# clovaai/assembled-cnn

Hardware: AMD Instinct MI355X
Metric: images/sec Assemble-ResNet-50 224^2 bf16 train (higher is better)
Workload: dtype bf16; 1 GPU; Assemble-ResNet-50 (BigLittle + SK + anti_alias sconv k=3 + resnet_d) bf16 train; per_gpu_batch=256, global_batch=256, image=224x224x3, num_classes=1001, parallelism=dp1

## Files before the change

### assembled_cnn_amd/csrc/conv_gemm1.hip

```cpp
#include "common.h"
#include "igemm_common.h"

using namespace asm_igemm;

namespace {

typedef __attribute__((address_space(3))) void* lptr_t;

template <int N>
__device__ __forceinline__ void wait_vm() {
  asm volatile("s_waitcnt vmcnt(%0)" ::"n"(N) : "memory");
}
template <int P, int RMAX>
__device__ __forceinline__ void wait_vm_steps(const int r) {
  if constexpr (RMAX <= 0) {
    wait_vm<0>();
  } else {
    if (r >= RMAX) wait_vm<P * RMAX>();
    else wait_vm_steps<P, RMAX - 1>(r);
  }
}

template <int BM, int BN, int BK, int WGM, int WGN, int NS>
struct Cfg1 {
  using C = Cfg<BM, BN, BK, WGM, WGN, false, true>;
  static constexpr int STAGE = (BM + BN) * C::ROWB;
  static constexpr int LDS = cmax(cmax(NS * STAGE, C::EPI), C::RED);
  static constexpr int P = C::XP + C::WP;
  static_assert(BN % C::RPP == 0, "every wave issues the same number of pieces (the vmcnt immediates count them)");
  static_assert(C::RPP % 16 == 0, "the source-side swizzle must not depend on the pass");
  static_assert(NS >= 2 && P * (NS - 2) <= 63, "vmcnt is a 6-bit counter");
  static_assert(LDS <= 160 * 1024, "lds");
};

template <int BM, int BN, int BK, int WGM, int WGN, bool STATS, int NS, bool PFA, bool POOL, bool BNRED = false>
__global__ __launch_bounds__(64 * WGM * WGN) void igemm1_kernel(IGemmArgs p) {
  using C = Cfg<BM, BN, BK, WGM, WGN, false, STATS>;
  using C1 = Cfg1<BM, BN, BK, WGM, WGN, NS>;
  constexpr int CPR = C::CPR, RPP = C::RPP, XP = C::XP, WP = C::WP, ROWB = C::ROWB, STAGE = C1::STAGE, P = C1::P;
  constexpr int TM = C::TM, TN = C::TN, WTM = C::WTM, WTN = C::WTN;
  constexpr int KK = BK / 16;
  static_assert(KK >= 2 && KK % 2 == 0, "fragment double buffer: the last group of a step lives in buffer 1");

  extern __shared__ __attribute__((aligned(16))) unsigned char smem[];

  const int tid = threadIdx.x;
  const int lane = tid & 63;
  const int wave = tid >> 6;
  const int wm = wave / WGN, wn = wave % WGN;

  int logical;
  {
    const int nb = p.n_blocks, q = nb >> 3, r = nb & 7;
    const int bid = blockIdx.x, xcd = bid & 7, idx = bid >> 3;
    logical = (xcd < r ? xcd * (q + 1) : r * (q + 1) + (xcd - r) * q) + idx;
  }
  const int tile_m = (int)fd_div((unsigned)logical, p.fd_ntn);
  const int tile_n = logical - tile_m * p.n_tiles_n;

  const __amdgpu_buffer_rsrc_t rx = make_rsrc(p.x, p.x_bytes);
  const __amdgpu_buffer_rsrc_t rw = make_rsrc(p.w, p.w_bytes);

  const int chunk = tid % CPR;
  const int r0 = tid / CPR;
  const int csw = (chunk ^ swz<BK>(r0)) << 3;
  const bool c_ok = csw < p.Ci;

  unsigned vx[XP];
#pragma unroll
  for (int j = 0; j < XP; ++j) {
    const int m = tile_m * BM + r0 + j * RPP;
    bool ok = c_ok && m < p.M;
    const unsigned img = fd_div((unsigned)m, p.fd_howo);
    const unsigned rem = (unsigned)m - img * (unsigned)p.HoWo;
    const unsigned ho = fd_div(rem, p.fd_wo);
    const unsigned wo = rem - ho * (unsigned)p.Wo;
    int nh = (int)ho * p.so - p.pad, nw = (int)wo * p.so - p.pad_w;
    if (p.sd == 2) {
      ok = ok && (((nh | nw) & 1) == 0);
      nh >>= 1;
      nw >>= 1;
    }
    ok = ok && ((unsigned)nh < (unsigned)p.Hi) && ((unsigned)nw < (unsigned)p.Wi);
    vx[j] = ok ? (img * (unsigned)p.x_img_pitch + (unsigned)nh * (unsigned)p.x_row_pitch +
                  (unsigned)nw * (unsigned)p.x_pix_pitch + (unsigned)csw) * 2u
               : ASM_OOB;
  }
  unsigned vw[WP];
#pragma unroll
  for (int j = 0; j < WP; ++j) {
    const int n = tile_n * BN + r0 + j * RPP;
    vw[j] = (c_ok && n < p.Co) ? ((unsigned)n * (unsigned)p.w_row_pitch + (unsigned)csw) * 2u : ASM_OOB;
  }

  const int wrow0 = wave * (64 / CPR);
  const unsigned wtap = (unsigned)p.wt0 * (unsigned)p.Ci * 2u;
  auto issue = [&](int stage, unsigned kb) {
    unsigned char* xs = smem + stage * STAGE;
    unsigned char* ws = xs + BM * ROWB;
#pragma unroll
    for (int j = 0; j < XP; ++j)
      __builtin_amdgcn_raw_ptr_buffer_load_lds(rx, (lptr_t)(xs + (j * RPP + wrow0) * ROWB), 16, (int)vx[j], (int)kb, 0, 0);
#pragma unroll
    for (int j = 0; j < WP; ++j)
      __builtin_amdgcn_raw_ptr_buffer_load_lds(rw, (lptr_t)(ws + (j * RPP + wrow0) * ROWB), 16, (int)vw[j],
                                               (int)(kb + wtap), 0, 0);
  };

  f32x16 acc[TN][TM];
#pragma unroll
  for (int a = 0; a < TN; ++a)
#pragma unroll
    for (int b = 0; b < TM; ++b)
#pragma unroll
      for (int i = 0; i < 16; ++i) acc[a][b][i] = 0.f;

  const int l31 = lane & 31, lhi = lane >> 5;
  unsigned fwo[KK], fxo[KK];
#pragma unroll
  for (int kk = 0; kk < KK; ++kk) {
    const int ch = kk * 2 + lhi;
    const int rw_ = wn * WTN + l31, rx_ = wm * WTM + l31;
    fwo[kk] = BM * ROWB + rw_ * ROWB + ((ch ^ swz<BK>(rw_)) << 4);
    fxo[kk] = rx_ * ROWB + ((ch ^ swz<BK>(rx_)) << 4);
  }
  bf16x8 fwb[2][TN], fxb[2][TM];
  auto load_frags = [&](int stage, const int kk, const int buf) {
    const unsigned char* sb = smem + stage * STAGE;
#pragma unroll
    for (int a = 0; a < TN; ++a) fwb[buf][a] = *reinterpret_cast<const bf16x8*>(sb + fwo[kk] + a * 32 * ROWB);
#pragma unroll
    for (int b = 0; b < TM; ++b) fxb[buf][b] = *reinterpret_cast<const bf16x8*>(sb + fxo[kk] + b * 32 * ROWB);
  };
  auto mma = [&](const int buf) {
#pragma unroll
    for (int a = 0; a < TN; ++a)
#pragma unroll
      for (int b = 0; b < TM; ++b)
        acc[a][b] = __builtin_amdgcn_mfma_f32_32x32x16_bf16(fwb[buf][a], fxb[buf][b], acc[a][b], 0, 0, 0);
  };

  const int nk = p.kchunks;
#pragma unroll
  for (int s = 0; s < NS - 1; ++s)
    if (s < nk) issue(s, (unsigned)(s * BK * 2));
#pragma unroll
  for (int a = 0; a < TN; ++a) fwb[1][a] = bf16x8{0, 0, 0, 0, 0, 0, 0, 0};
#pragma unroll
  for (int b = 0; b < TM; ++b) fxb[1][b] = bf16x8{0, 0, 0, 0, 0, 0, 0, 0};
  int cur = 0;
  unsigned kb_next = (unsigned)((NS - 1) * BK * 2);
#pragma unroll 1
  for (int kc = 0; kc < nk; ++kc) {
    wait_vm_steps<P, NS - 2>(nk - 1 - kc);
    asm volatile("s_waitcnt lgkmcnt(0)\n\ts_barrier" ::: "memory");
    load_frags(cur, 0, 0);
    mma(1);
    if (kc + NS - 1 < nk) {
      int nst = cur + NS - 1;
      if (nst >= NS) nst -= NS;
      issue(nst, kb_next);
    }
#pragma unroll
    for (int kk = 0; kk + 1 < KK; ++kk) {
      load_frags(cur, kk + 1, (kk + 1) & 1);
      mma(kk & 1);
    }
    cur = cur + 1 == NS ? 0 : cur + 1;
    kb_next += BK * 2;
  }
  mma(1);
  __syncthreads();

  igemm_epilogue<C, BM, BN, WTM, WTN, TM, TN, false, STATS, PFA, POOL, false, BNRED>(p, acc, smem, tile_m, tile_n, tid, wm, wn, l31, lhi);
}

template <int BM, int BN, int BK, int WGM, int WGN, bool STATS, int NS, bool PFA, bool POOL, bool BNRED = false>
int launch1_one(const IGemmArgs& a, hipStream_t st) {
  using C1 = Cfg1<BM, BN, BK, WGM, WGN, NS>;
  auto kern = igemm1_kernel<BM, BN, BK, WGM, WGN, STATS, NS, PFA, POOL, BNRED>;
  static bool attr_done[ASM_MAX_DEVICES] = {};
  if (hipError_t e = asm_ensure_dyn_lds(kern, C1::LDS, attr_done); e != hipSuccess)
    ASM_FAIL(ASM_EHIP, "igemm1_kernel: dynamic LDS opt-in: %s", hipGetErrorString(e));
  ASM_LAUNCH(kern, dim3(a.n_blocks), dim3(64 * WGM * WGN), C1::LDS, st, a);
  ASM_CHECK_LAUNCH("igemm1_kernel");
  return ASM_OK;
}

template <int BM, int BN, int BK, int WGM, int WGN, int NS>
int launch1(const ConvLaunch& L, const IGemmArgs& a, hipStream_t st) {
  switch (L.epi) {
    case EPI_BNRED: return launch1_one<BM, BN, BK, WGM, WGN, true, NS, false, false, true>(a, st);
    case EPI_STATS: return launch1_one<BM, BN, BK, WGM, WGN, true, NS, false, false>(a, st);
    case EPI_POOL: return launch1_one<BM, BN, BK, WGM, WGN, false, NS, false, true>(a, st);
    case EPI_PFA: return launch1_one<BM, BN, BK, WGM, WGN, false, NS, true, false>(a, st);
    case EPI_PLAIN: return launch1_one<BM, BN, BK, WGM, WGN, false, NS, false, false>(a, st);
  }
  return conv_no_variant("igemm1_kernel", L.epi);
}

struct Config {
  int code;
  ConvTile t;
  int (*launch)(const ConvLaunch&, const IGemmArgs&, hipStream_t);
};
constexpr Config kConfigs[] = {
    {1, {128, 128, 64, 2, 2}, launch1<128, 128, 64, 2, 2, 2>},
    {5, {128, 128, 32, 2, 2}, launch1<128, 128, 32, 2, 2, 3>},
    {8, {256, 128, 64, 4, 2}, launch1<256, 128, 64, 4, 2, 3>},
    {10, {128, 128, 32, 2, 2}, launch1<128, 128, 32, 2, 2, 2>},
    {11, {128, 64, 64, 2, 2}, launch1<128, 64, 64, 2, 2, 2>},
    {12, {128, 64, 32, 2, 2}, launch1<128, 64, 32, 2, 2, 3>},
    {13, {128, 64, 32, 2, 2}, launch1<128, 64, 32, 2, 2, 2>},
    {14, {256, 128, 32, 4, 2}, launch1<256, 128, 32, 4, 2, 3>},
    {16, {128, 256, 32, 2, 2}, launch1<128, 256, 32, 2, 2, 2>},
};

struct AutoRow {
  int kind, M, Ci, Co, code;
};
constexpr AutoRow kAuto[] = {
    {0, 802816,   32,   64, 13}, {0, 802816,   32,  128, 13}, {0, 802816,   64,   32, 12}, {0, 802816,   64,  128, 10},
    {0, 802816,  128,  256, 10}, {0, 802816,  256,   64, 12}, {0, 200704,   64,  256, 10}, {0, 200704,  256,   64, 12},
    {0, 200704,  256,  128,  5}, {0, 200704,  256,  256,  5}, {0, 200704,  256,  512, 10}, {0, 200704,  512,  128,  5},
    {0,  50176,  128,  512, 10}, {0,  50176,  256,  512, 10}, {0,  50176,  256, 1024, 10}, {0,  50176,  512,  128, 14},
    {0,  50176,  512,  256, 16}, {0,  50176,  512,  512, 10}, {0,  50176,  512, 1024, 10}, {0,  50176, 1024,  256, 16},
    {0,  50176, 1024,  512, 16}, {0,  50176, 1024, 1024, 14}, {0,  12544,  256, 1024, 16}, {0,  12544,  512, 1024, 14},
    {0,  12544,  512, 2048, 10}, {0,  12544, 1024,  256,  5}, {0,  12544, 2048,  512,  8}, {1, 802816,   32,   64, 12},
    {1, 802816,   64,   32, 12}, {1, 802816,   64,   64, 11}, {1, 802816,   64,  256, 16}, {1, 802816,  128,   32, 13},
    {1, 802816,  128,   64, 13}, {1, 802816,  256,  128,  5}, {1, 200704,   64,  256,  5}, {1, 200704,  128,  256,  5},
    {1, 200704,  128,  512,  5}, {1, 200704,  256,   64, 12}, {1, 200704,  256,  256, 10}, {1, 200704,  512,  256,  5},
    {1,  50176,  128,  512, 10}, {1,  50176,  256,  512, 10}, {1,  50176,  256, 1024, 14}, {1,  50176,  512,  128,  1},
    {1,  50176,  512,  512, 10}, {1,  50176,  512, 1024, 10}, {1,  50176, 1024,  256, 16}, {1,  50176, 1024,  512, 14},
    {1,  50176, 1024, 1024, 10}, {1,  12544,  256, 1024, 14}, {1,  12544,  512, 2048, 10}, {1,  12544, 1024,  256,  8},
    {1,  12544, 1024,  512,  8}, {1,  12544, 2048,  512,  8}, {1,  12544, 2048, 1024, 16}, {2, 802816,   64,  256, 14},
    {2, 200704,   64,  256, 13}, {2, 200704,  128,  256, 12}, {2, 200704,  128,  512, 14}, {2,  50176,  128,  512, 12},
    {2,  50176,  256,  512, 12}, {2,  50176,  256, 1024, 13}, {2,  50176,  512, 1024, 14}, {2,  12544,  256, 1024, 14},
    {2,  12544,  512, 2048, 14},
    {0, 802816,   64,  256, 10}, {1, 802816,  256,   64, 11}, {0, 802816,  256,  128, 14}, {1, 802816,  128,  256, 14},
    {2, 802816,  128,  256, 14}, {0, 200704,  128,  512, 10}, {1, 200704,  512,  128,  5}, {0, 200704,  512,  256,  5},
    {1, 200704,  256,  512, 10}, {2, 200704,  256,  512, 14}, {0, 401408,   64,   64, 12}, {1, 100352,  256,   64, 12},
    {0, 100352,  256,   64, 12}, {1, 100352,   64,  256,  5}, {2, 100352,   64,  256, 13}, {0, 401408,   64,  256, 10},
    {0, 401408,  256,  256,  5}, {1, 401408,  256,  256, 14}, {0, 100352,  256,  256, 10}, {1, 100352,  256,  256, 10},
    {0, 401408,  256,   64, 12}, {1, 401408,   64,  256,  5}, {2, 401408,   64,  256, 14}, {0,  25088,  256,  512, 16},
    {1,  25088,  512,  256,  8}, {0, 100352,  256,  128, 14}, {1, 100352,  128,  256, 12}, {2, 100352,  128,  256, 12},
    {0,  25088,  128,  512, 10}, {1,  25088,  512,  128, 11}, {0,  25088,  512,  128,  5}, {1,  25088,  128,  512, 14},
    {2,  25088,  128,  512, 12}, {0, 100352,  256,  512, 10}, {0, 100352,  128,  512, 10}, {1, 100352,  512,  128, 14},
    {1, 100352,  128,  512, 10}, {2, 100352,  128,  512, 12}, {0, 100352,  512,  512, 14}, {1, 100352,  512,  512, 14},
    {1,   6272, 1024,  512,  5}, {0,  25088,  512,  256,  8}, {1,  25088,  256,  512, 14}, {2,  25088,  256,  512, 14},
    {1,   6272, 1024,  256, 12}, {0,   6272, 1024,  256, 11}, {1,   6272,  256, 1024,  8}, {0,  25088,  256, 1024, 10},
    {1,  25088, 1024,  256,  8}, {0,  25088, 1024,  256,  8}, {1,  25088,  256, 1024, 10}, {2,  25088,  256, 1024, 10},
    {1,   6272, 2048, 1024,  8}, {1,   6272, 2048,  512,  5}, {0,   6272, 2048,  512,  5},
};

int auto_cfg(const IGemmArgs& a, bool stats) {
  if (a.so != 1 || a.sd != 1 || a.y_strided || a.pool_dy) return 0;
  const int kind = a.tsign < 0 ? (a.addend ? 2 : 1) : (stats ? 0 : -1);
  for (const AutoRow& r : kAuto)
    if (r.kind == kind && r.M == a.M && r.Ci == a.Ci && r.Co == a.Co) return r.code;
  return 0;
}

}

int asm_gemm1_config(const IGemmArgs& a, bool out_f32, bool stats, ConvTile* t) {
  if (out_f32 || a.R != 1 || a.S != 1 || a.bn_scale) return 0;
  const int g = asm_tune().gemm1;
  const int code = g < 0 ? auto_cfg(a, stats) : g;
  for (const Config& c : kConfigs)
    if (c.code == code && (a.Ci % c.t.bk == 0 || a.Ci <= c.t.bk)) { *t = c.t; return code; }
  return 0;
}

int asm_gemm1_launch(const ConvLaunch& L, const IGemmArgs& a, hipStream_t st) {
  for (const Config& c : kConfigs)
// ... 4 lines not shown
```

### assembled_cnn_amd/csrc/conv_igemm.hip

```cpp
#include "common.h"
#include "igemm_common.h"

using namespace asm_igemm;

int asm_gemm1_config(const IGemmArgs& a, bool out_f32, bool stats, ConvTile* t);
int asm_gemm1_launch(const ConvLaunch& L, const IGemmArgs& a, hipStream_t st);
bool asm_igemm8_covers(const IGemmArgs& a, bool out_f32);
int asm_igemm8_launch(const ConvLaunch& L, const IGemmArgs& a, hipStream_t st);

namespace {

__device__ __attribute__((aligned(16))) unsigned g_zero16[4] = {0u, 0u, 0u, 0u};


template <int BM, int BN, int BK, int WGM, int WGN, bool OUT_F32, bool STATS, bool BNRED = false>
__global__ __launch_bounds__(64 * WGM * WGN) void igemm_kernel(IGemmArgs p) {
  using C = Cfg<BM, BN, BK, WGM, WGN, OUT_F32, STATS>;
  constexpr int NT = C::NT, CPR = C::CPR, RPP = C::RPP, XP = C::XP, WP = C::WP, ROWB = C::ROWB, STAGE = C::STAGE;
  constexpr int TM = C::TM, TN = C::TN, WTM = C::WTM, WTN = C::WTN;

  extern __shared__ __attribute__((aligned(16))) unsigned char smem[];

  const int tid = threadIdx.x;
  const int lane = tid & 63;
// ... 72 lines not shown
    const int tap0 = (kt_r * p.S + kt_s) * p.Ci + kt_c * BK;
#pragma unroll
    for (int j = 0; j < WP; ++j) {
      const int row = r0 + j * RPP;
      if (j * RPP + wrow0 < BN) {
        const int c = ((chunk ^ swz<BK>(row)) << 3);
        const bool ok = live && (kt_c * BK + c < p.Ci) && (wb[j] >= 0);
        const unsigned off = (unsigned)(wb[j] + tap0 + c) * 2u;
        const unsigned char* src = ok ? reinterpret_cast<const unsigned char*>(p.w) + off
                                      : reinterpret_cast<const unsigned char*>(g_zero16);
        __builtin_amdgcn_global_load_lds((gptr_t)src, (lptr_t)(ws + (j * RPP + wrow0) * ROWB), 16, 0, 0);
      }
    }
    if (++kt_s == p.S) {
      kt_s = 0;
      if (++kt_r == p.R) {
        kt_r = 0;
        ++kt_c;
      }
    }
  };

  f32x16 acc[TN][TM];
#pragma unroll
  for (int a = 0; a < TN; ++a)
#pragma unroll
    for (int b = 0; b < TM; ++b)
#pragma unroll
      for (int i = 0; i < 16; ++i) acc[a][b][i] = 0.f;

  const int KT = p.R * p.S * p.kchunks;
  const int l31 = lane & 31, lhi = lane >> 5;

  auto compute = [&](int stage) {
    const unsigned char* xs = smem + stage * STAGE;
    const unsigned char* ws = xs + BM * ROWB;
#pragma unroll
    for (int kk = 0; kk < BK / 16; ++kk) {
      const int ch = kk * 2 + lhi;
      bf16x8 fw[TN], fx[TM];
#pragma unroll
      for (int a = 0; a < TN; ++a) {
        const int row = wn * WTN + a * 32 + l31;
        fw[a] = *reinterpret_cast<const bf16x8*>(ws + row * ROWB + ((ch ^ swz<BK>(row)) << 4));
      }
#pragma unroll
      for (int b = 0; b < TM; ++b) {
        const int row = wm * WTM + b * 32 + l31;
        fx[b] = *reinterpret_cast<const bf16x8*>(xs + row * ROWB + ((ch ^ swz<BK>(row)) << 4));
      }
#pragma unroll
      for (int a = 0; a < TN; ++a)
#pragma unroll
        for (int b = 0; b < TM; ++b)
          acc[a][b] = __builtin_amdgcn_mfma_f32_32x32x16_bf16(fw[a], fx[b], acc[a][b], 0, 0, 0);
    }
  };

  issue_tile(0, true);
  asm volatile("s_waitcnt vmcnt(0)" ::: "memory");
  __syncthreads();
#pragma unroll 1
  for (int kt = 0; kt < KT; ++kt) {
    const int cur = kt & 1;
    if (kt + 1 < KT) issue_tile(cur ^ 1, true);
    compute(cur);
    asm volatile("s_waitcnt vmcnt(0)" ::: "memory");
    __syncthreads();
  }

  igemm_epilogue<C, BM, BN, WTM, WTN, TM, TN, OUT_F32, STATS, false, false, false, BNRED>(p, acc, smem, tile_m, tile_n, tid, wm, wn, l31, lhi);
}

template <int BM, int BN, int BK, int WGM, int WGN, bool OUT_F32, bool STATS, int NS>
struct Cfg2 {
  using C = Cfg<BM, BN, BK, WGM, WGN, OUT_F32, STATS>;
  static constexpr int WROWS = BN;
  static constexpr int STAGE = (BM + WROWS) * C::ROWB;
  static constexpr int LDS = cmax(cmax(NS * STAGE, C::EPI), C::RED);
  static_assert(LDS <= 160 * 1024, "lds");
};

template <int BM, int BN, int BK, int WGM, int WGN, bool OUT_F32, bool STATS, int R, int S, int NS, bool PFA = false, bool POOL = false,
          int SCHED = 0, bool BNRED = false>
__global__ __launch_bounds__(64 * WGM * WGN) void igemm2_kernel(IGemmArgs p) {
  using C = Cfg<BM, BN, BK, WGM, WGN, OUT_F32, STATS>;
  using C2 = Cfg2<BM, BN, BK, WGM, WGN, OUT_F32, STATS, NS>;
  constexpr int CPR = C::CPR, RPP = C::RPP, XP = C::XP, WP = C::WP, ROWB = C::ROWB, STAGE = C2::STAGE;
  constexpr int TM = C::TM, TN = C::TN, WTM = C::WTM, WTN = C::WTN;
  constexpr int NTAP = R * S;
  static_assert(RPP % 16 == 0, "the source-side swizzle must not depend on the pass");
  typedef __attribute__((address_space(3))) void* lptr_t;

  extern __shared__ __attribute__((aligned(16))) unsigned char smem[];

  const int tid = threadIdx.x;
  const int lane = tid & 63;
  const int wave = tid >> 6;
  const int wm = wave / WGN, wn = wave % WGN;

  int logical;
  {
    const int nb = p.n_blocks, q = nb >> 3, r = nb & 7;
    const int bid = blockIdx.x, xcd = bid & 7, idx = bid >> 3;
    logical = (xcd < r ? xcd * (q + 1) : r * (q + 1) + (xcd - r) * q) + idx;
  }
  const int tile_m0 = (int)fd_div((unsigned)logical, p.fd_ntn);
  const int tile_n = logical - tile_m0 * p.n_tiles_n;
  const int tile_m = tile_m0 + p.m_tile0;

  const __amdgpu_buffer_rsrc_t rx = make_rsrc(p.x, p.x_bytes);
  const __amdgpu_buffer_rsrc_t rw = make_rsrc(p.w, p.w_bytes);

  const int chunk = tid % CPR;
  const int r0 = tid / CPR;
  const int csw = (chunk ^ swz<BK>(r0)) << 3;
  const bool c_ok = csw < p.Ci;

  unsigned vx[XP][NTAP];
#pragma unroll
  for (int j = 0; j < XP; ++j) {
    const int m = tile_m * BM + r0 + j * RPP;
    const bool live = c_ok && m < p.M;
    const unsigned img = fd_div((unsigned)m, p.fd_howo);
    const unsigned rem = (unsigned)m - img * (unsigned)p.HoWo;
    const unsigned ho = fd_div(rem, p.fd_wo);
    const unsigned wo = rem - ho * (unsigned)p.Wo;
    const int bh = (int)ho * p.so - p.pad, bw = (int)wo * p.so - p.pad_w;
    const unsigned base = img * (unsigned)p.x_img_pitch + (unsigned)csw;
    unsigned roff[R], coff[S];
    bool rok[R], cok[S];
#pragma unroll
    for (int r = 0; r < R; ++r) {
      int nh = bh + p.tsign * r;
      bool ok = live;
      if (p.sd == 2) {
        ok = ok && ((nh & 1) == 0);
        nh >>= 1;
      }
      rok[r] = ok && ((unsigned)nh < (unsigned)p.Hi);
      roff[r] = base + (unsigned)nh * (unsigned)p.x_row_pitch;
    }
#pragma unroll
    for (int q = 0; q < S; ++q) {
      int nw = bw + p.tsign * q;
      bool ok = true;
      if (p.sd == 2) {
        ok = ((nw & 1) == 0);
        nw >>= 1;
      }
      cok[q] = ok && ((unsigned)nw < (unsigned)p.Wi);
      coff[q] = (unsigned)nw * (unsigned)p.x_pix_pitch;
    }
#pragma unroll
    for (int r = 0; r < R; ++r)
#pragma unroll
      for (int q = 0; q < S; ++q) vx[j][r * S + q] = (rok[r] && cok[q]) ? (roff[r] + coff[q]) * 2u : ASM_OOB;
  }
  unsigned vw[WP];
#pragma unroll
  for (int j = 0; j < WP; ++j) {
    const int row = r0 + j * RPP;
    const int n = tile_n * BN + row;
    vw[j] = (c_ok && row < BN && n < p.Co) ? ((unsigned)n * (unsigned)p.w_row_pitch + (unsigned)csw) * 2u : ASM_OOB;
  }

  const int wrow0 = wave * (64 / CPR);
// ... 407 lines not shown
  };

  unsigned fxo[TM], fwo[TN];
#pragma unroll
  for (int b = 0; b < TM; ++b) {
    const int row = wm * WTM + b * 32 + l31;
    fxo[b] = (unsigned)(((row >> 4) * HW_ + (row & 15)) * RB + lhi * 16);
  }
#pragma unroll
  for (int a = 0; a < TN; ++a) fwo[a] = (unsigned)((wn * WTN + a * 32 + l31) * WROWB);
  const int wsw = swz<CI>(wn * WTN + l31);

  u32x4 hv[HP];
  if (t_begin < t_end) load_halo(t_begin, hv);
  asm volatile("s_waitcnt vmcnt(0)" ::: "memory");

#pragma unroll 1
  for (int tile = t_begin; tile < t_end; ++tile) {
    __syncthreads();
    store_halo(hv);
    __syncthreads();
    if (tile + 1 < t_end) load_halo(tile + 1, hv);

    f32x16 acc[TN][TM];
#pragma unroll
    for (int a = 0; a < TN; ++a)
#pragma unroll
      for (int b = 0; b < TM; ++b)
#pragma unroll
        for (int i = 0; i < 16; ++i) acc[a][b][i] = 0.f;
#pragma unroll
    for (int t = 0; t < 9; ++t) {
      const int r = t / 3, q = t - r * 3;
      const int hoff = (p.tsign > 0 ? (r * HW_ + q) : ((2 - r) * HW_ + (2 - q))) * RB;
#pragma unroll
      for (int kk = 0; kk < KK; ++kk) {
        bf16x8 fw[TN], fx[TM];
#pragma unroll
        for (int a = 0; a < TN; ++a)
          fw[a] = *reinterpret_cast<const bf16x8*>(ws + t * WTAP + fwo[a] + (((kk * 2 + lhi) ^ wsw) << 4));
#pragma unroll
        for (int b = 0; b < TM; ++b) fx[b] = *reinterpret_cast<const bf16x8*>(xs + fxo[b] + hoff + kk * 32);
#pragma unroll
        for (int a = 0; a < TN; ++a)
#pragma unroll
          for (int b = 0; b < TM; ++b) acc[a][b] = __builtin_amdgcn_mfma_f32_32x32x16_bf16(fw[a], fx[b], acc[a][b], 0, 0, 0);
      }
    }
    __syncthreads();
    const int img = tile / tpi, trem = tile - img * tpi;
    const int ty = trem / tiles_x, tx = trem - ty * tiles_x;
    const int patch_base = (img * p.Hi + ty * 8) * p.Wi + tx * 16;
    igemm_epilogue<C, 128, KO, WTM, WTN, TM, TN, false, STATS>(p, acc, xs, tile, 0, tid, wm, wn, l31, lhi, patch_base);
  }
}

template <int KO, int CI, int WGM, int WGN, bool STATS>
int launch_halo_one(const IGemmArgs& a, hipStream_t st) {
  using H = HaloCfg<KO, CI>;
  auto kern = conv_halo_kernel<KO, CI, WGM, WGN, STATS>;
  static bool attr_done[ASM_MAX_DEVICES] = {};
  if (hipError_t e = asm_ensure_dyn_lds(kern, H::LDS, attr_done); e != hipSuccess)
    ASM_FAIL(ASM_EHIP, "conv_halo_kernel: dynamic LDS opt-in: %s", hipGetErrorString(e));
  ASM_LAUNCH(kern, dim3(a.n_blocks), dim3(256), H::LDS, st, a);
  ASM_CHECK_LAUNCH("conv_halo_kernel");
  return ASM_OK;
}

template <int KO, int CI, int WGM, int WGN>
int launch_halo(const ConvLaunch& L, const IGemmArgs& a, hipStream_t st) {
  return L.epi == EPI_STATS ? launch_halo_one<KO, CI, WGM, WGN, true>(a, st) : launch_halo_one<KO, CI, WGM, WGN, false>(a, st);
}

bool halo_covers(const IGemmArgs& a, bool out_f32) {
  if (out_f32 || a.R != 3 || a.S != 3 || a.so != 1 || a.sd != 1 || a.y_strided || a.bn_scale) return false;
  if (a.Hi % 8 || a.Wi % 16 || a.M != (a.HoWo / a.Wo) * a.Wo * (a.M / a.HoWo) || a.HoWo != a.Hi * a.Wi) return false;
  if (a.x_pix_pitch != a.Ci || a.x_row_pitch != a.Wi * a.Ci || a.x_img_pitch != a.Hi * a.Wi * a.Ci) return false;
  if (!((a.tsign > 0 && a.pad == 1 && a.pad_w == 1) || (a.tsign < 0 && a.pad == -1 && a.pad_w == -1))) return false;
  if (a.wt0 != 0 || a.wtr != 3 || a.wts != 1) return false;
  return (a.Ci == 32 || a.Ci == 64) && (a.Co == 32 || a.Co == 64);
}

template <int BM, int BN, int BK, int WGM, int WGN, bool OUT_F32, bool STATS, int R, int S, int NS = 2, bool PFA = false, bool POOL = false,
          int SCHED = 0, bool BNRED = false>
int launch2_one(const IGemmArgs& a, hipStream_t st) {
  using C = Cfg2<BM, BN, BK, WGM, WGN, OUT_F32, STATS, NS>;
  constexpr int NTHR = 64 * WGM * WGN;
  if constexpr (SCHED == 0 && BK == 64 && BN >= 128 && !OUT_F32 && !POOL && ((R == 3 && S == 3) || (R == 1 && S == 1))) {
    if (R == 3) return launch2_one<BM, BN, BK, WGM, WGN, OUT_F32, STATS, R, S, NS, PFA, POOL, 1>(a, st);
  }
  auto kern = igemm2_kernel<BM, BN, BK, WGM, WGN, OUT_F32, STATS, R, S, NS, PFA, POOL, SCHED, BNRED>;
  static bool attr_done[ASM_MAX_DEVICES] = {};
  if (hipError_t e = asm_ensure_dyn_lds(kern, C::LDS, attr_done); e != hipSuccess)
    ASM_FAIL(ASM_EHIP, "igemm2_kernel: dynamic LDS opt-in: %s", hipGetErrorString(e));
  ASM_LAUNCH(kern, dim3(a.n_blocks), dim3(NTHR), C::LDS, st, a);
  ASM_CHECK_LAUNCH("igemm2_kernel");
  return ASM_OK;
}

constexpr unsigned igemm2_variants(int R, int S, int BM, int BN, int BK) {
  if (R == 1 && S == 1)
    return epi_bit(EPI_F32) | epi_bit(EPI_BNRED) | epi_bit(EPI_STATS) | epi_bit(EPI_POOL) | epi_bit(EPI_PFA) | epi_bit(EPI_PLAIN);
  if (R == 3 && S == 3) return epi_bit(EPI_STATS) | epi_bit(EPI_PFA) | epi_bit(EPI_PLAIN);
  if ((R == 1 && S == 2) || (R == 2 && S == 1) || (R == 2 && S == 2)) return epi_bit(EPI_PLAIN);
  if ((R == 7 || R == 3) && S == 1 && BK == 32 && BM == 128 && BN <= 64) return epi_bit(EPI_STATS) | epi_bit(EPI_PLAIN);
  return 0;
}

template <int BM, int BN, int BK, int WGM, int WGN, int R, int S>
int launch2_rs(const ConvLaunch& L, const IGemmArgs& a, hipStream_t st) {
  constexpr unsigned has = igemm2_variants(R, S, BM, BN, BK);
  if constexpr ((has >> EPI_F32) & 1)
    if (L.epi == EPI_F32) return launch2_one<BM, BN, BK, WGM, WGN, true, false, R, S>(a, st);
  if constexpr ((has >> EPI_BNRED) & 1)
    if (L.epi == EPI_BNRED) return launch2_one<BM, BN, BK, WGM, WGN, false, true, R, S, 2, false, false, 0, true>(a, st);
  if constexpr ((has >> EPI_STATS) & 1)
    if (L.epi == EPI_STATS) return launch2_one<BM, BN, BK, WGM, WGN, false, true, R, S>(a, st);
  if constexpr ((has >> EPI_POOL) & 1)
    if (L.epi == EPI_POOL) return launch2_one<BM, BN, BK, WGM, WGN, false, false, R, S, 2, false, true>(a, st);
  if constexpr ((has >> EPI_PFA) & 1)
    if (L.epi == EPI_PFA) return launch2_one<BM, BN, BK, WGM, WGN, false, false, R, S, 2, true>(a, st);
  if constexpr ((has >> EPI_PLAIN) & 1)
    if (L.epi == EPI_PLAIN) return launch2_one<BM, BN, BK, WGM, WGN, false, false, R, S>(a, st);
  return conv_no_variant("igemm2_kernel", L.epi);
}

template <int BM, int BN, int BK, int WGM, int WGN>
struct Launch2 {
  static int run(const ConvLaunch& L, const IGemmArgs& a, hipStream_t st) {
    if (a.R == 1 && a.S == 1) return launch2_rs<BM, BN, BK, WGM, WGN, 1, 1>(L, a, st);
    if (a.R == 3 && a.S == 3) return launch2_rs<BM, BN, BK, WGM, WGN, 3, 3>(L, a, st);
    if (a.R == 1 && a.S == 2) return launch2_rs<BM, BN, BK, WGM, WGN, 1, 2>(L, a, st);
    if (a.R == 2 && a.S == 1) return launch2_rs<BM, BN, BK, WGM, WGN, 2, 1>(L, a, st);
    if (a.R == 2 && a.S == 2) return launch2_rs<BM, BN, BK, WGM, WGN, 2, 2>(L, a, st);
    if (a.R == 7 && a.S == 1) return launch2_rs<BM, BN, BK, WGM, WGN, 7, 1>(L, a, st);
    if (a.R == 3 && a.S == 1) return launch2_rs<BM, BN, BK, WGM, WGN, 3, 1>(L, a, st);
    return conv_no_variant("igemm2_kernel", L.epi);
  }
};

template <int BM, int BN, int BK, int WGM, int WGN, bool OUT_F32, bool STATS, bool BNRED = false>
int launch_one(const IGemmArgs& a, hipStream_t st) {
  using C = Cfg<BM, BN, BK, WGM, WGN, OUT_F32, STATS>;
  auto kern = igemm_kernel<BM, BN, BK, WGM, WGN, OUT_F32, STATS, BNRED>;
  static bool attr_done[ASM_MAX_DEVICES] = {};
  if (hipError_t e = asm_ensure_dyn_lds(kern, C::LDS, attr_done); e != hipSuccess)
    ASM_FAIL(ASM_EHIP, "igemm_kernel: dynamic LDS opt-in: %s", hipGetErrorString(e));
  ASM_LAUNCH(kern, dim3(a.n_blocks), dim3(C::NT), C::LDS, st, a);
  ASM_CHECK_LAUNCH("igemm_kernel");
  return ASM_OK;
}

template <int BM, int BN, int BK, int WGM, int WGN>
struct LaunchGeneral {
  static int run(const ConvLaunch& L, const IGemmArgs& a, hipStream_t st) {
    switch (L.epi) {
      case EPI_F32: return launch_one<BM, BN, BK, WGM, WGN, true, false>(a, st);
      case EPI_BNRED: return launch_one<BM, BN, BK, WGM, WGN, false, true, true>(a, st);
      case EPI_STATS: return launch_one<BM, BN, BK, WGM, WGN, false, true>(a, st);
      case EPI_PLAIN: return launch_one<BM, BN, BK, WGM, WGN, false, false>(a, st);
    }
    return conv_no_variant("igemm_kernel", L.epi);
  }
};

template <template <int, int, int, int, int> class F>
int on_tile(const ConvLaunch& L, const IGemmArgs& a, hipStream_t st) {
  const ConvTile& t = L.t;
  if (t.bm == 256) return F<256, 256, 64, 4, 2>::run(L, a, st);
  if (t.bn == 32) return t.bk == 64 ? F<128, 32, 64, 4, 1>::run(L, a, st) : F<128, 32, 32, 4, 1>::run(L, a, st);
  if (t.bn == 64) return t.bk == 64 ? F<128, 64, 64, 2, 2>::run(L, a, st) : F<128, 64, 32, 2, 2>::run(L, a, st);
  return t.bk == 64 ? F<128, 128, 64, 2, 2>::run(L, a, st) : F<128, 128, 32, 2, 2>::run(L, a, st);
}

enum class ConvOut { bf16, f32, stats, bnred };

bool tile256(const IGemmArgs& a) {
  const int ftile = asm_tune().igemm_tile;
  if (ftile == 1) return false;
  if (ftile == 3 && a.Ci % 64 == 0) return true;
  const long long b256 = (long long)cdiv(a.M, 256) * cdiv(a.Co, 256);
  return a.Ci % 64 == 0 && (long long)a.R * a.S * a.Ci >= 512 && a.Co >= 256 && b256 >= 192;
}

ConvTile pick_tile(const IGemmArgs& a) {
  const long long t128 = (long long)cdiv(a.M, 128) * cdiv(a.Co, 128);
  const bool bk64 = a.Ci % 64 == 0 && (a.R * a.S > 1 || (a.Ci >= 256 && t128 <= 4000));
  if (a.Co <= 32) return bk64 ? ConvTile{128, 32, 64, 4, 1} : ConvTile{128, 32, 32, 4, 1};
  if (a.Co <= 64) return bk64 ? ConvTile{128, 64, 64, 2, 2} : ConvTile{128, 64, 32, 2, 2};
  if (tile256(a)) return ConvTile{256, 256, 64, 4, 2};
  return bk64 ? ConvTile{128, 128, 64, 2, 2} : ConvTile{128, 128, 32, 2, 2};
}

unsigned family_variants(int family, const IGemmArgs& a, const ConvTile& t) {
  switch (family) {
    case FAM_GENERAL: return epi_bit(EPI_F32) | epi_bit(EPI_BNRED) | epi_bit(EPI_STATS) | epi_bit(EPI_PLAIN);
    case FAM_IGEMM2: return igemm2_variants(a.R, a.S, t.bm, t.bn, t.bk);
    case FAM_HALO: return epi_bit(EPI_STATS) | epi_bit(EPI_PLAIN);
    case FAM_DENSE: return epi_bit(EPI_F32) | epi_bit(EPI_PLAIN);
    case FAM_GEMM1: return epi_bit(EPI_BNRED) | epi_bit(EPI_STATS) | epi_bit(EPI_POOL) | epi_bit(EPI_PFA) | epi_bit(EPI_PLAIN);
    default: return epi_bit(EPI_BNRED) | epi_bit(EPI_STATS) | epi_bit(EPI_PFA) | epi_bit(EPI_PLAIN);
  }
}

ConvLaunch tiled(int family, ConvTile t, const IGemmArgs& a, ConvOut out, int M, int m_tile0) {
  ConvLaunch L = {};
  L.family = family; L.t = t; L.M = M; L.m_tile0 = m_tile0;
  L.n_tiles_n = cdiv(a.Co, t.bn);
  L.n_blocks = (cdiv(M, t.bm) - m_tile0) * L.n_tiles_n;
  L.kchunks = cdiv(a.Ci, t.bk);
  const unsigned has = family_variants(family, a, t);
  const int pfa_env = asm_tune().igemm_pfa;
  const bool pfa = (has & epi_bit(EPI_PFA)) && a.addend != nullptr && !a.y_strided &&
                   (pfa_env >= 0 ? pfa_env != 0 : (t.bm == 256 || L.n_blocks <= 1024));
  const int want = out == ConvOut::f32 ? EPI_F32 : out == ConvOut::bnred ? EPI_BNRED : out == ConvOut::stats ? EPI_STATS
                   : a.pool_dy ? EPI_POOL : pfa ? EPI_PFA : EPI_PLAIN;
  L.epi = (has & epi_bit(want)) ? want : -1;
  if (family == FAM_IGEMM3) {
    L.nhb = a.Ci == 64 ? 1 : 2;
    L.hr = a.Ci == 64 && a.Wi > 30 ? 256 : 192;
  }
  return L;
}

ConvPlan single(const ConvLaunch& L) { return ConvPlan{1, {L, {}}, nullptr}; }
ConvPlan no_plan(const char* why) { return ConvPlan{0, {}, why}; }

bool dense_shaped(const IGemmArgs& a) {
  return a.Hi == 1 && a.Wi == 1 && a.HoWo == 1 && a.R == 1 && a.S == 1 && a.x_img_pitch == a.Ci && a.x_row_pitch == a.Ci &&
         a.x_pix_pitch == a.Ci;
}
bool dense_covers(const IGemmArgs& a, ConvOut out) {
  if (!asm_tune().dense_small || !dense_shaped(a) || a.Ci % 16 || (out != ConvOut::bf16 && out != ConvOut::f32)) return false;
  if (a.addend_mask || a.pool_dy || a.bn_scale || a.y_strided) return false;
  if (a.ldy % 4 || a.ldy > cdiv(a.Co, 32) * 32) return false;
  return asm_aligned16(a.x) && asm_aligned16(a.w) && asm_aligned16(a.y) && asm_aligned16(a.addend);
}

ConvPlan plan_conv(const IGemmArgs& a, ConvOut out) {
  const asm_tuning& tu = asm_tune();
  const bool f32 = out == ConvOut::f32, stats = out == ConvOut::stats || out == ConvOut::bnred;
  const bool k1 = a.R == 1 && a.S == 1;
  const bool bnred3 = out == ConvOut::bnred && !k1;
  if (dense_covers(a, out)) return single(tiled(FAM_DENSE, ConvTile{32, 32, 16, 1, 1}, a, out, a.M, 0));
  if (dense_shaped(a) && (a.pool_dy || out == ConvOut::bnred))
    return no_plan("conv dgrad: the fused input-gradient forms do not take a [N,1,1,C] layer");
  if (a.pool_dy && (tu.igemm_mode != 0 || out != ConvOut::bf16 || !k1 || a.y_strided))
    return no_plan("conv dgrad_pooled: only the 1x1 stride-1 igemm2 path folds an average-pool backward in");
  if (tu.igemm_mode == 0 && tu.igemm_tile == 0) {
    if (halo_covers(a, f32)) {
      if (bnred3) return no_plan("conv dgrad_bnred: no kernel with the batch-norm sums for this 3x3 layer");
      const int ko = a.Co, ci = a.Ci;
      ConvLaunch L = tiled(FAM_HALO, ConvTile{128, ko, ci, ko == 32 ? 4 : 2, ko == 32 ? 1 : 2}, a, out, a.M, 0);
      const int per_cu = ko == 32 ? (ci == 32 ? HaloCfg<32, 32>::PER_CU : HaloCfg<32, 64>::PER_CU)
                                  : (ci == 32 ? HaloCfg<64, 32>::PER_CU : HaloCfg<64, 64>::PER_CU);
      L.n_blocks = a.M / 128 < per_cu * 256 ? a.M / 128 : per_cu * 256;
      return single(L);
    }
    ConvTile t1;
    if (const int code = asm_gemm1_config(a, f32, stats, &t1)) {
      ConvLaunch L = tiled(FAM_GEMM1, t1, a, out, a.M, 0);
      L.gemm1 = code;
      return single(L);
    }
    const int h3 = tu.igemm3, h8 = tu.igemm8;
    const ConvTile t128 = {128, 128, 64, 2, 2};
    const bool big = tile256(a);
    const long long b256 = (long long)cdiv(a.M, 256) * cdiv(a.Co, 256);
    const bool to_igemm3 = h3 && b256 >= 768 && a.Ci <= 128;
    const bool cov3 = h3 && igemm3_covers(a, f32);
    if (((h8 == 1 && big && !to_igemm3) || h8 == 2) && asm_igemm8_covers(a, f32)) {
      const ConvTile t8 = {256, 256, 64, 2, 4};
      const int cus = asm_num_cus();
      const int nt8 = cdiv(a.Co, 256), mt8 = cdiv(a.M, 256);
      const long long n8 = (long long)nt8 * mt8;
      const int m_full = (int)((n8 / cus) * cus / nt8);
      const long long rem = n8 - (long long)m_full * nt8;
      const double small = 4 * rem <= cus ? 0.3 : 0.5 * (double)((4 * rem + 2 * cus - 1) / (2 * cus));
      const double split_cost = (double)((long long)m_full * nt8 / cus) + small, whole_cost = (double)((n8 + cus - 1) / cus);
      if (h8 == 1 && m_full > 0 && rem > 0 && split_cost < whole_cost - 0.15 && (cov3 || !bnred3)) {
        return ConvPlan{2, {tiled(FAM_IGEMM8, t8, a, out, m_full * 256, 0),
                            tiled(cov3 ? FAM_IGEMM3 : FAM_IGEMM2, t128, a, out, a.M, m_full * 2)},
                        nullptr};
      }
      return single(tiled(FAM_IGEMM8, t8, a, out, a.M, 0));
    }
    if (cov3 && (h3 == 2 || !big || to_igemm3)) return single(tiled(FAM_IGEMM3, t128, a, out, a.M, 0));
  }
  if (bnred3) return no_plan("conv dgrad_bnred: no kernel with the batch-norm sums for this 3x3 layer");
  const ConvTile t = pick_tile(a);
  if (tu.igemm_mode == 0) {
    const ConvLaunch L = tiled(FAM_IGEMM2, t, a, out, a.M, 0);
    if (L.epi >= 0 && (a.Ci % t.bk == 0 || a.Ci <= t.bk)) return single(L);
    if (a.pool_dy) return no_plan("conv dgrad_pooled: no igemm2 instantiation for this shape");
  }
  return single(tiled(FAM_GENERAL, t, a, out, a.M, 0));
}

int run_plan(const ConvPlan& p, IGemmArgs a, hipStream_t st) {
  if (p.n == 0) ASM_FAIL(ASM_ENOTSUP, "%s", p.why);
  a.fd_howo = make_fastdiv((unsigned)a.HoWo);
  a.fd_wo = make_fastdiv((unsigned)a.Wo);
  for (int i = 0; i < p.n; ++i) {
    const ConvLaunch& L = p.l[i];
    a.M = L.M; a.m_tile0 = L.m_tile0; a.n_tiles_n = L.n_tiles_n; a.n_blocks = L.n_blocks; a.kchunks = L.kchunks;
    a.fd_ntn = make_fastdiv((unsigned)L.n_tiles_n);
    int rc;
    switch (L.family) {
      case FAM_GENERAL: rc = on_tile<LaunchGeneral>(L, a, st); break;
      case FAM_GEMM1: rc = asm_gemm1_launch(L, a, st); break;
      case FAM_IGEMM2: rc = on_tile<Launch2>(L, a, st); break;
      case FAM_IGEMM3: rc = L.nhb == 2 ? launch3<192, 2>(L, a, st) : L.hr == 192 ? launch3<192, 1>(L, a, st) : launch3<256, 1>(L, a, st); break;
      case FAM_HALO:
        rc = L.t.bn == 32 ? (L.t.bk == 64 ? launch_halo<32, 64, 4, 1>(L, a, st) : launch_halo<32, 32, 4, 1>(L, a, st))
                          : (L.t.bk == 64 ? launch_halo<64, 64, 2, 2>(L, a, st) : launch_halo<64, 32, 2, 2>(L, a, st));
        break;
      case FAM_IGEMM8: rc = asm_igemm8_launch(L, a, st); break;
      case FAM_DENSE:
        rc = asm_dense_small_launch(a.x, a.Ci, a.w, a.Ci, a.M, a.Co, a.Ci, a.y, a.ldy, L.epi == EPI_F32, a.addend, st);
        break;
      default: ASM_FAIL(ASM_EINVAL, "conv: no kernel family %d", L.family);
    }
    if (rc != ASM_OK) return rc;
  }
  asm_last_conv_kernel = p.l[p.n - 1].family;
  return ASM_OK;
}

int check_desc(const asm_conv_desc* d) {
  ASM_REQUIRE(d != nullptr, "conv: null descriptor");
  ASM_REQUIRE(d->N > 0 && d->H > 0 && d->W > 0 && d->C > 0 && d->K > 0 && d->R > 0 && d->S > 0,
              "conv: non-positive dimension");
  ASM_REQUIRE(d->C % 8 == 0, "conv: C=%d must be a multiple of 8", d->C);
  ASM_REQUIRE(d->stride == 1 || d->stride == 2, "conv: stride %d not supported", d->stride);
  ASM_REQUIRE(d->Ho > 0 && d->Wo > 0, "conv: bad output size");
  ASM_REQUIRE(d->pad >= 0 && d->pad < 64, "conv: bad pad");
  return ASM_OK;
}

}

static inline int64_t img_pitch(const asm_conv_desc* d) {
  return d->x_img_pitch ? d->x_img_pitch : (int64_t)d->H * d->W * d->C;
}
static inline int row_pitch(const asm_conv_desc* d) { return d->x_row_pitch ? d->x_row_pitch : d->W * d->C; }
static inline int pix_pitch(const asm_conv_desc* d) { return d->x_pix_pitch ? d->x_pix_pitch : d->C; }

extern "C" int asm_debug_last_conv_kernel(void) { return asm_last_conv_kernel; }

extern "C" int asm_conv2d_stats_blocks(const asm_conv_desc* d) {
  if (!d) return ASM_EINVAL;
  return cdiv(d->N * d->Ho * d->Wo, STATS_BM);
}

static int fprop_impl(const asm_conv_desc* d, const void* x, const void* w, void* y, float* stats_partial,
                      const float* bn_scale, const float* bn_shift, const void* residual, int relu, void* stream) {
  if (int e = check_desc(d)) return e;
  ASM_REQUIRE(x && w && y, "conv fprop: null pointer");
  const int64_t xelems = (int64_t)d->N * img_pitch(d);
  ASM_REQUIRE(xelems * 2 < (int64_t)ASM_OOB, "conv fprop: input larger than 2 GiB");
  const int ldy = d->ldy ? d->ldy : d->K;
  ASM_REQUIRE(ldy % (d->out_f32 ? 4 : 8) == 0 && ldy >= d->K, "conv fprop: bad ldy %d", ldy);
  ASM_REQUIRE(!(stats_partial && d->out_f32), "conv fprop: fused statistics need bf16 output");
  IGemmArgs a = {};
  a.x = x; a.w = w; a.y = y; a.addend = residual; a.stats = stats_partial;
  a.x_bytes = (unsigned)(xelems * 2);
  a.w_bytes = (unsigned)((int64_t)d->K * d->R * d->S * d->C * 2);
  a.M = d->N * d->Ho * d->Wo;
  a.Hi = d->H; a.Wi = d->W; a.Ci = d->C;
  a.Wo = d->Wo; a.HoWo = d->Ho * d->Wo;
  a.Co = d->K; a.ldy = ldy;
  a.R = d->R; a.S = d->S;
  a.so = d->stride; a.sd = 1; a.tsign = 1; a.pad = d->pad;
  a.pad_w = a.pad; a.wt0 = 0; a.wtr = a.S; a.wts = 1;
  a.bn_scale = bn_scale; a.bn_shift = bn_shift; a.bn_relu = relu;
  a.x_img_pitch = (int)img_pitch(d); a.x_row_pitch = row_pitch(d); a.x_pix_pitch = pix_pitch(d);
  a.w_row_pitch = d->R * d->S * d->C;
  const ConvOut out = d->out_f32 ? ConvOut::f32 : stats_partial ? ConvOut::stats : ConvOut::bf16;
  return run_plan(plan_conv(a, out), a, (hipStream_t)stream);
}

extern "C" int asm_conv2d_fprop(const asm_conv_desc* d, const void* x, const void* w, void* y,
                                float* stats_partial, void* stream) {
  return fprop_impl(d, x, w, y, stats_partial, nullptr, nullptr, nullptr, 0, stream);
}

extern "C" int asm_conv2d_fprop_bn(const asm_conv_desc* d, const void* x, const void* w, void* y, const float* scale,
                                   const float* shift, const void* residual, int relu, void* stream) {
  ASM_REQUIRE(d && scale && shift, "conv fprop_bn: null pointer");
  ASM_REQUIRE(!d->out_f32 && d->K % 8 == 0, "conv fprop_bn: needs bf16 output and K %% 8 == 0 (K=%d)", d->K);
  ASM_REQUIRE(d->ldy == 0 || d->ldy == d->K, "conv fprop_bn: padded output rows not supported");
  return fprop_impl(d, x, w, y, nullptr, scale, shift, residual, relu ? 1 : 0, stream);
}

struct PoolAdd {
  const void* dy;
  int k, stride, pad, Hp, Wp, cv;
};
struct BnRed {
  const void* y;
  const uint8_t* mask;
  float* partial;
};
static int dgrad_impl(const asm_conv_desc* d, const void* dy, const void* wt, const void* addend,
                      const uint8_t* addend_mask, void* dx, void* stream, const PoolAdd* pool = nullptr,
                      const BnRed* red = nullptr);
static IGemmArgs dgrad_args(const asm_conv_desc* d) {
  IGemmArgs a = {};
  a.x_bytes = (unsigned)((int64_t)d->N * d->Ho * d->Wo * d->K * 2);
  a.w_bytes = (unsigned)((int64_t)d->K * d->R * d->S * d->C * 2);
  a.M = d->N * d->H * d->W;
  a.Hi = d->Ho; a.Wi = d->Wo; a.Ci = d->K;
  a.Wo = d->W; a.HoWo = d->H * d->W;
  a.Co = d->C; a.ldy = d->C;
  a.R = d->R; a.S = d->S;
  a.so = 1; a.sd = d->stride; a.tsign = -1; a.pad = -d->pad; a.pad_w = a.pad;
  a.x_img_pitch = d->Ho * d->Wo * d->K; a.x_row_pitch = d->Wo * d->K; a.x_pix_pitch = d->K;
  a.w_row_pitch = d->R * d->S * d->K;
  a.wt0 = 0; a.wtr = a.S; a.wts = 1;
  return a;
}
static int dgrad_check(const asm_conv_desc* d) {
  if (int e = check_desc(d)) return e;
  ASM_REQUIRE(d->K % 8 == 0, "conv dgrad: K=%d must be a multiple of 8 (pad dy)", d->K);
  ASM_REQUIRE(d->x_img_pitch == 0 && d->x_row_pitch == 0 && d->x_pix_pitch == 0 && !d->out_f32,
              "conv dgrad: custom pitches / f32 output not supported");
  const int64_t dyelems = (int64_t)d->N * d->Ho * d->Wo * d->K;
  ASM_REQUIRE(dyelems * 2 < (int64_t)ASM_OOB, "conv dgrad: dy larger than 2 GiB");
  return ASM_OK;
}
bool asm_dgrad_s2_covers(const asm_conv_desc* d);
int asm_dgrad_s2_launch(const asm_conv_desc* d, const void* dy, const void* wt, const void* addend, const uint8_t* addend_mask,
                        void* dx, void* stream);

enum class DgradForm { conv, parity, s2 };
struct DgradPlan {
  DgradForm form;
  int nc;
  IGemmArgs cls[4];
  ConvPlan cp[4];
  bool fill;
  ConvPlan conv;
};

static DgradPlan plan_dgrad(const asm_conv_desc* d, const IGemmArgs& a, ConvOut out, bool aligned) {
  DgradPlan p = {};
  const asm_tuning& tu = asm_tune();
  const bool k3 = d->R == 3 && d->S == 3, k1 = d->R == 1 && d->S == 1 && d->pad == 0;
  if (dense_covers(a, out)) {
    p.conv = plan_conv(a, out);
    return p;
  }
  if (aligned && !a.pool_dy && asm_dgrad_s2_covers(d)) {
    p.form = DgradForm::s2;
    return p;
  }
  if (tu.dgrad_parity && d->stride == 2 && (k3 || k1) && tu.igemm_mode == 0) {
    if (k1 && a.addend_mask) {
      p.conv = no_plan("conv dgrad_masked: a masked addend is not supported for the 1x1 stride-2 input gradient");
      return p;
    }
    for (int cls = 0; cls < 4; ++cls) {
      const int ph = cls >> 1, pw = cls & 1;
      const int Hc = (d->H - ph + 1) / 2, Wc = (d->W - pw + 1) / 2;
      const int r0 = (ph + d->pad) & 1, s0 = (pw + d->pad) & 1;
      const int Rc = (d->R - r0 + 1) / 2, Sc = (d->S - s0 + 1) / 2;
      if (Hc <= 0 || Wc <= 0 || Rc <= 0 || Sc <= 0) continue;
      IGemmArgs& c = p.cls[p.nc];
      c = a;
      c.R = Rc; c.S = Sc;
      c.M = d->N * Hc * Wc;
      c.Wo = Wc; c.HoWo = Hc * Wc;
      c.so = 1; c.sd = 1; c.tsign = -1;
      c.pad = -((ph + d->pad - r0) / 2); c.pad_w = -((pw + d->pad - s0) / 2);
      c.wt0 = r0 * d->S + s0; c.wtr = 2 * d->S; c.wts = 2;
      c.y_strided = 1;
      c.y_base = (ph * d->W + pw) * d->C;
      c.y_img_pitch = d->H * d->W * d->C; c.y_row_pitch = 2 * d->W * d->C; c.y_pix_pitch = 2 * d->C;
      p.cp[p.nc] = plan_conv(c, ConvOut::bf16);
      if (p.cp[p.nc].n > 0 && p.cp[p.nc].l[0].family == FAM_GENERAL) {
        p.nc = 0;
        break;
      }
      ++p.nc;
    }
    if (p.nc > 0) {
      p.form = DgradForm::parity;
      p.fill = k1;
      return p;
    }
  }
  p.conv = plan_conv(a, out);
  return p;
}

extern "C" int asm_conv2d_dgrad(const asm_conv_desc* d, const void* dy, const void* wt, const void* addend,
                                void* dx, void* stream) {
  return dgrad_impl(d, dy, wt, addend, nullptr, dx, stream);
}

extern "C" int asm_conv2d_dgrad_masked(const asm_conv_desc* d, const void* dy, const void* wt, const void* addend,
                                       const uint8_t* addend_mask, void* dx, void* stream) {
  ASM_REQUIRE(addend && addend_mask, "conv dgrad_masked: needs the addend and its mask");
  ASM_REQUIRE(d && d->C % 8 == 0, "conv dgrad_masked: C must be a multiple of 8");
  return dgrad_impl(d, dy, wt, addend, addend_mask, dx, stream);
}

extern "C" int asm_conv2d_dgrad_pooled(const asm_conv_desc* d, const void* dy, const void* wt, const void* addend,
                                       const uint8_t* addend_mask, const void* pool_dy, int pool_k, int pool_stride,
                                       int pool_pad, int pool_Ho, int pool_Wo, int count_valid, void* dx, void* stream) {
  ASM_REQUIRE(d && pool_dy, "conv dgrad_pooled: null pointer");
  ASM_REQUIRE(d->R == 1 && d->S == 1 && d->stride == 1 && d->pad == 0 && d->C % 8 == 0,
              "conv dgrad_pooled: needs a 1x1 stride-1 convolution with C %% 8 == 0");
  ASM_REQUIRE(pool_k >= 1 && (pool_stride == 1 || pool_stride == 2) && pool_pad >= 0 && pool_Ho > 0 && pool_Wo > 0,
              "conv dgrad_pooled: bad pooling geometry");
  if (pool_k > 2 * pool_stride || pool_k < pool_stride)
    ASM_FAIL(ASM_ENOTSUP, "conv dgrad_pooled: window %d / stride %d puts a pixel in more than two windows per dimension",
             pool_k, pool_stride);
  ASM_REQUIRE(!addend_mask || addend, "conv dgrad_pooled: a mask needs its addend");
  const PoolAdd pa = {pool_dy, pool_k, pool_stride, pool_pad, pool_Ho, pool_Wo, count_valid ? 1 : 0};
  return dgrad_impl(d, dy, wt, addend, addend_mask, dx, stream, &pa);
}

static bool dgrad_bnred_covers(const asm_conv_desc* d) {
  if (!d || d->C % 8 || d->K % 8 || d->stride != 1 || d->x_img_pitch || d->x_row_pitch || d->x_pix_pitch || d->out_f32) return false;
  if (!(d->R == 1 && d->S == 1 && d->pad == 0) && !(d->R == 3 && d->S == 3 && d->pad == 1 && d->Ho == d->H && d->Wo == d->W))
    return false;
  const ConvPlan p = plan_conv(dgrad_args(d), ConvOut::bnred);
  for (int i = 0; i < p.n; ++i)
    if (p.l[i].epi != EPI_BNRED) return false;
  return p.n > 0;
}

extern "C" int asm_conv2d_dgrad_bnred_blocks(const asm_conv_desc* d) {
  if (!d) return ASM_EINVAL;
  if (!dgrad_bnred_covers(d)) return 0;
  return cdiv(d->N * d->H * d->W, STATS_BM);
}

extern "C" int asm_conv2d_dgrad_bnred(const asm_conv_desc* d, const void* dy, const void* wt, const void* addend,
                                      const uint8_t* addend_mask, const void* bn_y, const uint8_t* bn_relu_mask,
                                      float* partial, void* dx, void* stream) {
  ASM_REQUIRE(d && bn_y && partial, "conv dgrad_bnred: null pointer");
  ASM_REQUIRE(!addend_mask || addend, "conv dgrad_bnred: a mask needs its addend");
  if (!dgrad_bnred_covers(d))
    ASM_FAIL(ASM_ENOTSUP, "conv dgrad_bnred: 1x1 stride-1 layers, and the 3x3 stride-1 layers of the igemm8 / igemm3 kernels, with "
             "C %% 8 == 0 only (%dx%d, stride %d, C %d)", d->R, d->S, d->stride, d->C);
  const BnRed r = {bn_y, bn_relu_mask, partial};
  return dgrad_impl(d, dy, wt, addend, addend_mask, dx, stream, nullptr, &r);
}

extern "C" int asm_conv2d_dgrad_kernel(const asm_conv_desc* d, int variant) {
  if (int e = dgrad_check(d)) return e;
  ASM_REQUIRE(!(variant & ~(ASM_DGRAD_MASKED | ASM_DGRAD_POOLED | ASM_DGRAD_BNRED)), "conv dgrad_kernel: bad variant %d", variant);
  const bool pooled = variant & ASM_DGRAD_POOLED, bnred = variant & ASM_DGRAD_BNRED;
  if (pooled && (bnred || d->R != 1 || d->S != 1 || d->stride != 1 || d->pad != 0))
    ASM_FAIL(ASM_ENOTSUP, "conv dgrad_kernel: the pooled input gradient is a 1x1 stride-1 one without the batch-norm sums");
  if (bnred && !dgrad_bnred_covers(d)) ASM_FAIL(ASM_ENOTSUP, "conv dgrad_kernel: no batch-norm sums for this layer");
  alignas(16) static const unsigned char operand[16] = {};
  IGemmArgs a = dgrad_args(d);
  if (variant & ASM_DGRAD_MASKED) {
    a.addend = operand;
    a.addend_mask = operand;
  }
  if (pooled) a.pool_dy = operand;
  const DgradPlan p = plan_dgrad(d, a, bnred ? ConvOut::bnred : ConvOut::bf16, true);
  if (p.form == DgradForm::s2) return FAM_DGRAD_S2;
  const ConvPlan& last = p.form == DgradForm::parity ? p.cp[p.nc - 1] : p.conv;
  if (last.n == 0) ASM_FAIL(ASM_ENOTSUP, "%s", last.why);
  return last.l[last.n - 1].family;
}

static int dgrad_impl(const asm_conv_desc* d, const void* dy, const void* wt, const void* addend,
                      const uint8_t* addend_mask, void* dx, void* stream, const PoolAdd* pool, const BnRed* red) {
  if (int e = dgrad_check(d)) return e;
  ASM_REQUIRE(dy && wt && dx, "conv dgrad: null pointer");
  IGemmArgs a = dgrad_args(d);
  a.x = dy; a.w = wt; a.y = dx; a.addend = addend; a.addend_mask = addend_mask;
  if (red) {
    a.stats = red->partial; a.red_y = red->y; a.red_mask = red->mask;
  }
  if (pool) {
    a.pool_dy = pool->dy; a.pool_k = pool->k; a.pool_stride = pool->stride; a.pool_pad = pool->pad;
    a.pool_Hp = pool->Hp; a.pool_Wp = pool->Wp; a.pool_cv = pool->cv; a.pool_H = d->H;
  }
  const bool aligned = ((reinterpret_cast<uintptr_t>(dy) | reinterpret_cast<uintptr_t>(wt) | reinterpret_cast<uintptr_t>(dx) |
                         reinterpret_cast<uintptr_t>(addend)) & 15) == 0;
  const DgradPlan p = plan_dgrad(d, a, red ? ConvOut::bnred : ConvOut::bf16, aligned);
  const hipStream_t st = (hipStream_t)stream;
  switch (p.form) {
    case DgradForm::s2:
      if (const int rc = asm_dgrad_s2_launch(d, dy, wt, addend, addend_mask, dx, stream)) return rc;
      asm_last_conv_kernel = FAM_DGRAD_S2;
      return ASM_OK;
    case DgradForm::parity:
      if (p.fill) {
        const size_t bytes = (size_t)a.M * d->C * 2;
        hipError_t e = (addend && addend != dx) ? asm_fill_async(dx, addend, 0, bytes, st)
                     : addend ? hipSuccess
                              : asm_fill_async(dx, nullptr, 0, bytes, st);
        if (e != hipSuccess) ASM_FAIL(ASM_EHIP, "conv dgrad: fill: %s", hipGetErrorString(e));
      }
      for (int i = 0; i < p.nc; ++i)
        if (const int rc = run_plan(p.cp[i], p.cls[i], st)) return rc;
      return ASM_OK;
    case DgradForm::conv: break;
  }
  return run_plan(p.conv, a, st);
}
```

### assembled_cnn_amd/csrc/igemm_common.h

```cpp
#pragma once
#include "common.h"

static inline bool asm_dense_shaped(const asm_conv_desc* d) {
  return d->H == 1 && d->W == 1 && d->Ho == 1 && d->Wo == 1 && d->R == 1 && d->S == 1 && d->C % 8 == 0 &&
         (d->x_img_pitch == 0 || d->x_img_pitch == d->C) && (d->x_row_pitch == 0 || d->x_row_pitch == d->C) &&
         (d->x_pix_pitch == 0 || d->x_pix_pitch == d->C);
}
int asm_dense_small_launch(const void* p, int ldp, const void* q, int ldq, int M, int N, int K, void* out, int ldo, bool out_f32,
                           const void* addend, hipStream_t st);
int asm_dense_small_wgrad_launch(const void* x, int ldx, const void* dy, int ldy, int M, int Cin, int Cout, float* dw, int ldw,
                                 hipStream_t st);
static inline bool asm_aligned16(const void* p) { return (reinterpret_cast<uintptr_t>(p) & 15u) == 0; }

namespace asm_igemm {

struct IGemmArgs {
  const void* x;
  const void* w;
  void* y;
  const void* addend;
  const uint8_t* addend_mask;
  float* stats;
  unsigned x_bytes, w_bytes;
  int M;
  int Hi, Wi, Ci;
  int Wo, HoWo;
  int Co;
  int ldy;
  int R, S;
  int so, sd, tsign, pad;
  int x_img_pitch, x_row_pitch, x_pix_pitch;
  int w_row_pitch;
  int n_tiles_n, n_blocks, kchunks;
  int m_tile0;
  FastDiv fd_howo, fd_wo, fd_ntn;
  int pad_w;
  int wt0, wtr, wts;
  int y_strided;
  int y_base, y_img_pitch, y_row_pitch, y_pix_pitch;
  const float* bn_scale;
  const float* bn_shift;
  int bn_relu;
  const void* red_y;
  const uint8_t* red_mask;
  const void* pool_dy;
  int pool_k, pool_stride, pool_pad, pool_Hp, pool_Wp, pool_cv, pool_H;
};

constexpr int STATS_BM = 128;

enum ConvFamily { FAM_GENERAL = 0, FAM_GEMM1 = 1, FAM_IGEMM2 = 2, FAM_IGEMM3 = 3, FAM_HALO = 4, FAM_DGRAD_S2 = 5, FAM_DENSE = 6, FAM_IGEMM8 = 8 };
enum ConvEpi { EPI_PLAIN, EPI_PFA, EPI_POOL, EPI_STATS, EPI_BNRED, EPI_F32 };
constexpr unsigned epi_bit(int e) { return 1u << e; }
struct ConvTile {
  int bm, bn, bk, wgm, wgn;
};
struct ConvLaunch {
  int family;
  int epi;
  ConvTile t;
  int gemm1;
  int hr, nhb;
  int M, m_tile0;
  int n_tiles_n, n_blocks, kchunks;
};
struct ConvPlan {
  int n;
  ConvLaunch l[2];
  const char* why;
};
static inline int conv_no_variant(const char* kernel, int epi) { ASM_FAIL(ASM_EINVAL, "conv: %s has no epilogue variant %d", kernel, epi); }

template <int BK>
__device__ __forceinline__ int swz(int row) {
  return BK == 64 ? ((row >> 1) & 7) : ((row >> 2) & 3);
}

constexpr int cmax(int a, int b) { return a > b ? a : b; }

template <int BM, int BN, int BK, int WGM, int WGN, bool OUT_F32, bool STATS>
struct Cfg {
  static constexpr int NT = 64 * WGM * WGN;
  static constexpr int CPR = BK / 8;
  static constexpr int RPP = NT / CPR;
  static constexpr int XP = BM / RPP;
  static constexpr int WP = cmax(1, BN / RPP);
  static constexpr int ROWB = BK * 2;
  static constexpr int STAGE = (BM + BN) * ROWB;
  static constexpr int WTM = BM / WGM, WTN = BN / WGN;
  static constexpr int TM = WTM / 32, TN = WTN / 32;
  static constexpr int LDO = BN * 2 + 16;
  static constexpr int CPO = BN / 8;
  static constexpr int RPO = NT / CPO;
  static constexpr int OP = BM / RPO;
  static constexpr int EPI = OUT_F32 ? 0 : BM * LDO;
  static constexpr int RED = STATS ? RPO * BN * 2 * 4 : 0;
  static constexpr int LDS = cmax(cmax(2 * STAGE, EPI), RED);
  static_assert(BM % RPP == 0 && (BN % RPP == 0 || BN < RPP), "loader tiling");
  static_assert(WTM % 32 == 0 && WTN % 32 == 0 && BM % RPO == 0, "wave tiling");
  static_assert(LDS <= 160 * 1024, "lds");
  static_assert(!STATS || BM % STATS_BM == 0, "stats granularity");
};

template <class C, int BM, int BN, int WTM, int WTN, int TM, int TN, bool OUT_F32, bool STATS, bool PFA = false, bool POOL = false,
          bool SPLIT8 = false, bool BNRED = false, int RPF = 1>
__device__ __forceinline__ void igemm_epilogue(const IGemmArgs& p, f32x16 (&acc)[TN][TM], unsigned char* smem,
                                               int tile_m, int tile_n, int tid, int wm, int wn, int l31, int lhi,
                                               int patch_base = -1) {
  if constexpr (OUT_F32) {
    static_assert(!SPLIT8, "igemm8 writes bf16");
    float* y = reinterpret_cast<float*>(p.y);
    const int co4 = (p.Co + 3) & ~3;
#pragma unroll
    for (int a = 0; a < TN; ++a)
#pragma unroll
      for (int b = 0; b < TM; ++b) {
        const int m = tile_m * BM + wm * WTM + b * 32 + l31;
        if (m < p.M) {
#pragma unroll
          for (int g = 0; g < 4; ++g) {
            const int n = tile_n * BN + wn * WTN + a * 32 + 8 * g + 4 * lhi;
            if (n < co4) {
              f32x4 v = {acc[a][b][4 * g], acc[a][b][4 * g + 1], acc[a][b][4 * g + 2], acc[a][b][4 * g + 3]};
              *reinterpret_cast<f32x4*>(y + (size_t)m * p.ldy + n) = v;
            }
          }
        }
      }
  } else {
    constexpr int LDO = C::LDO, CPO = C::CPO, RPO = C::RPO, OP = C::OP;
    unsigned char* os = smem;
    bf16_t* y = reinterpret_cast<bf16_t*>(p.y);
    const int oc = tid % CPO, orow = tid / CPO;
    const int n0 = tile_n * BN + oc * 8;
    const int co8 = (p.Co + 7) & ~7;
    auto row_off = [&](int row, int m) -> size_t {
      if (patch_base >= 0) return (size_t)(patch_base + (row >> 4) * p.Wi + (row & 15)) * p.ldy + n0;
      if (p.y_strided) {
        const unsigned img = fd_div((unsigned)m, p.fd_howo);
        const unsigned rem = (unsigned)m - img * (unsigned)p.HoWo;
        const unsigned ho = fd_div(rem, p.fd_wo);
        const unsigned wo = rem - ho * (unsigned)p.Wo;
        return (size_t)p.y_base + (size_t)img * p.y_img_pitch + (size_t)ho * p.y_row_pitch + (size_t)wo * p.y_pix_pitch + n0;
      }
      return (size_t)m * p.ldy + n0;
    };
    constexpr bool PF_ON = PFA && !STATS;
    constexpr int PF = !PF_ON ? 1 : (OP < 8 ? OP : 8);
    u32x4 av[PF];
    unsigned amk[PF];
    auto prefetch = [&](int ps0) {
#pragma unroll
      for (int i = 0; i < PF; ++i) {
        const int row = (ps0 + i) * RPO + orow;
        const int m = tile_m * BM + row;
        const bool ok = m < p.M && n0 < co8;
        const size_t yo = row_off(row, ok ? m : 0);
        const u32x4 z4 = {0u, 0u, 0u, 0u};
        av[i] = ok ? *reinterpret_cast<const u32x4*>(reinterpret_cast<const bf16_t*>(p.addend) + yo) : z4;
        amk[i] = (ok && p.addend_mask) ? (unsigned)p.addend_mask[yo >> 3] : 0xffu;
      }
    };
    if constexpr (PF_ON) {
      if (p.addend) prefetch(0);
    }
#pragma unroll
    for (int a = 0; a < TN; ++a)
#pragma unroll
      for (int b = 0; b < TM; ++b) {
        const int ml = SPLIT8 ? (b >> 1) * 128 + wm * 64 + (b & 1) * 32 + l31 : wm * WTM + b * 32 + l31;
#pragma unroll
        for (int g = 0; g < 4; ++g) {
          const int nl = SPLIT8 ? a * 128 + wn * 32 + 8 * g + 4 * lhi : wn * WTN + a * 32 + 8 * g + 4 * lhi;
          u32x2 v;
          v.x = pack2bf(acc[a][b][4 * g], acc[a][b][4 * g + 1]);
          v.y = pack2bf(acc[a][b][4 * g + 2], acc[a][b][4 * g + 3]);
          *reinterpret_cast<u32x2*>(os + ml * LDO + nl * 2) = v;
        }
      }
    __syncthreads();
    struct PoolTaps {
      u32x4 v[4];
      float w[4];
    };
    PoolTaps pcur, pnxt;
    auto pool_issue = [&](int ps, PoolTaps& t) {
      const int row = ps * RPO + orow;
      const int m = tile_m * BM + row;
      const bool ok = m < p.M && n0 < co8;
      const unsigned mm = ok ? (unsigned)m : 0u;
      const unsigned img = fd_div(mm, p.fd_howo);
      const unsigned rem = mm - img * (unsigned)p.HoWo;
      const unsigned ph = fd_div(rem, p.fd_wo);
      const unsigned pw = rem - ph * (unsigned)p.Wo;
      const int H = p.pool_H, W = p.Wo;
      const int sh = p.pool_stride >> 1;
      const int th = (int)ph + p.pool_pad, tw = (int)pw + p.pool_pad;
      int oh[2], ow[2];
      float wh[2], ww[2];
      oh[0] = th >> sh; ow[0] = tw >> sh;
      oh[1] = oh[0] - 1; ow[1] = ow[0] - 1;
      const int rh = th - (oh[0] << sh), rw = tw - (ow[0] << sh);
      bool vh[2], vw[2];
      vh[0] = ok && oh[0] < p.pool_Hp;           vw[0] = ow[0] < p.pool_Wp;
      vh[1] = ok && oh[1] >= 0 && oh[1] < p.pool_Hp && rh + p.pool_stride <= p.pool_k - 1;
      vw[1] = ow[1] >= 0 && ow[1] < p.pool_Wp && rw + p.pool_stride <= p.pool_k - 1;
#pragma unroll
      for (int i = 0; i < 2; ++i) {
        float ch_ = (float)p.pool_k, cw_ = (float)p.pool_k;
        if (p.pool_cv) {
          int a_ = 0, b_ = 0;
          for (int q = 0; q < p.pool_k; ++q) {
            a_ += ((unsigned)(oh[i] * p.pool_stride + q - p.pool_pad) < (unsigned)H);
            b_ += ((unsigned)(ow[i] * p.pool_stride + q - p.pool_pad) < (unsigned)W);
          }
          ch_ = (float)(a_ > 0 ? a_ : 1);
          cw_ = (float)(b_ > 0 ? b_ : 1);
        }
        wh[i] = vh[i] ? 1.0f / ch_ : 0.f;
        ww[i] = vw[i] ? 1.0f / cw_ : 0.f;
        oh[i] = vh[i] ? oh[i] : 0;
        ow[i] = vw[i] ? ow[i] : 0;
      }
      const bf16_t* src = reinterpret_cast<const bf16_t*>(p.pool_dy) + (size_t)img * p.pool_Hp * p.pool_Wp * p.ldy +
                          (n0 < co8 ? n0 : 0);
#pragma unroll
      for (int i = 0; i < 2; ++i)
#pragma unroll
        for (int j = 0; j < 2; ++j) {
          t.v[i * 2 + j] = *reinterpret_cast<const u32x4*>(src + (size_t)(oh[i] * p.pool_Wp + ow[j]) * p.ldy);
          t.w[i * 2 + j] = wh[i] * ww[j];
        }
    };
    if constexpr (POOL) pool_issue(0, pcur);
    constexpr int SG = STATS ? BM / STATS_BM : 1;
    float s[SG][8], ss[SG][8];
#pragma unroll
    for (int q = 0; q < SG; ++q)
#pragma unroll
      for (int e = 0; e < 8; ++e) s[q][e] = ss[q][e] = 0.f;
    static_assert(!BNRED || STATS, "the batch-norm backward sums use the statistics epilogue");
    constexpr int RD = !BNRED ? 1 : (RPF < OP ? RPF : OP);
    u32x4 ryv[RD];
    unsigned rmkv[RD];
    auto red_fetch = [&](int ps_, u32x4& yv, unsigned& mk) {
      const int row = ps_ * RPO + orow;
      const int m = tile_m * BM + row;
      const u32x4 z4 = {0u, 0u, 0u, 0u};
      yv = z4;
      mk = 0xffu;
      if (m < p.M && n0 < co8) {
        const size_t ro = row_off(row, m);
        yv = *reinterpret_cast<const u32x4*>(reinterpret_cast<const bf16_t*>(p.red_y) + ro);
        if (p.red_mask) mk = (unsigned)p.red_mask[ro >> 3];
      }
    };
    if constexpr (BNRED) {
#pragma unroll
      for (int i = 0; i < RD; ++i) red_fetch(i, ryv[i], rmkv[i]);
    }
#pragma unroll
    for (int ps = 0; ps < OP; ++ps) {
      if constexpr (PF_ON) {
        if (p.addend && ps > 0 && ps % PF == 0) prefetch(ps);
      }
      if constexpr (POOL) {
        if (ps + 1 < OP) pool_issue(ps + 1, pnxt);
      }
      const int row = ps * RPO + orow;
      const int m = tile_m * BM + row;
      u32x4 ry = ryv[ps % RD];
      unsigned rmk = rmkv[ps % RD];
      if constexpr (BNRED) {
        if (ps + RD < OP) red_fetch(ps + RD, ryv[ps % RD], rmkv[ps % RD]);
      }
      u32x4 v = *reinterpret_cast<const u32x4*>(os + row * LDO + oc * 16);
      if (m < p.M && n0 < co8) {
        const size_t yoff = row_off(row, m);
        if (POOL || p.addend || p.bn_scale) {
          float fv[8];
          unpack8(v, fv);
          if constexpr (POOL) {
#pragma unroll
            for (int t = 0; t < 4; ++t) {
              float g[8];
              unpack8(pcur.v[t], g);
#pragma unroll
              for (int e = 0; e < 8; ++e) fv[e] += g[e] * pcur.w[t];
            }
          }
          if (p.bn_scale) {
            const f32x4 s0 = *reinterpret_cast<const f32x4*>(p.bn_scale + n0), s1 = *reinterpret_cast<const f32x4*>(p.bn_scale + n0 + 4);
            const f32x4 h0 = *reinterpret_cast<const f32x4*>(p.bn_shift + n0), h1 = *reinterpret_cast<const f32x4*>(p.bn_shift + n0 + 4);
#pragma unroll
            for (int e = 0; e < 4; ++e) {
              fv[e] = fv[e] * s0[e] + h0[e];
              fv[e + 4] = fv[e + 4] * s1[e] + h1[e];
            }
          }
          if (p.addend) {
            if constexpr (!PF_ON) {
              av[0] = *reinterpret_cast<const u32x4*>(reinterpret_cast<const bf16_t*>(p.addend) + yoff);
              amk[0] = p.addend_mask ? (unsigned)p.addend_mask[yoff >> 3] : 0xffu;
            }
            float fa[8];
            unpack8(av[ps % PF], fa);
            const unsigned mk = amk[ps % PF];
#pragma unroll
            for (int e = 0; e < 8; ++e) fv[e] += ((mk >> e) & 1u) ? fa[e] : 0.f;
          }
          if (p.bn_relu) {
#pragma unroll
            for (int e = 0; e < 8; ++e) fv[e] = fmaxf(fv[e], 0.f);
          }
          v = pack8(fv);
        }
        *reinterpret_cast<u32x4*>(y + yoff) = v;
      }
      if constexpr (POOL) pcur = pnxt;
      if constexpr (STATS) {
        constexpr int PPG = OP / SG;
        float f[8];
        unpack8(v, f);
        if constexpr (BNRED) {
          float fy[8];
          unpack8(ry, fy);
#pragma unroll
          for (int e = 0; e < 8; ++e) {
            const float dz = ((rmk >> e) & 1u) ? f[e] : 0.f;
            s[ps / PPG][e] += dz;
            ss[ps / PPG][e] += dz * fy[e];
          }
        } else {
#pragma unroll
          for (int e = 0; e < 8; ++e) {
            s[ps / PPG][e] += f[e];
            ss[ps / PPG][e] += f[e] * f[e];
          }
        }
      }
    }
    if constexpr (STATS) {
      float* red = reinterpret_cast<float*>(smem);
#pragma unroll
      for (int q = 0; q < SG; ++q) {
        __syncthreads();
#pragma unroll
        for (int e = 0; e < 8; ++e) {
          red[(orow * 2 + 0) * BN + oc * 8 + e] = s[q][e];
          red[(orow * 2 + 1) * BN + oc * 8 + e] = ss[q][e];
        }
        __syncthreads();
        for (int idx = tid; idx < 2 * BN; idx += C::NT) {
          const int which = idx / BN, nl = idx - which * BN;
          float t = 0.f;
#pragma unroll 8
          for (int g = 0; g < RPO; ++g) t += red[(g * 2 + which) * BN + nl];
          const int n = tile_n * BN + nl;
          const int mb = tile_m * SG + q;
          if (n < p.Co && mb * STATS_BM < p.M) p.stats[((size_t)mb * 2 + which) * p.Co + n] = t;
        }
      }
    }
  }
}

}
```

### assembled_cnn_amd/lib.py

```python
from __future__ import annotations

import ctypes as C
import os

HERE = os.path.dirname(os.path.abspath(__file__))
LIB_PATH = os.environ.get('ASM_HIP_LIB') or os.path.join(HERE, 'libasm_hip.so')

ASM_OK, ASM_EINVAL, ASM_ENOTSUP, ASM_EHIP = 0, -1, -2, -3
ABI_VERSION = 11


class AsmError(RuntimeError):
  pass


class ImageDesc(C.Structure):
  _fields_ = [('src_offset', C.c_int64), ('Hs', C.c_int32), ('Ws', C.c_int32),
              ('crop_y', C.c_int32), ('crop_x', C.c_int32), ('crop_h', C.c_int32), ('crop_w', C.c_int32),
              ('resize_h', C.c_int32), ('resize_w', C.c_int32), ('out_y', C.c_int32), ('out_x', C.c_int32),
              ('flip', C.c_int32), ('reserved', C.c_int32)]


assert C.sizeof(ImageDesc) == 56

# ... 13 lines not shown
      (n, C.c_int32) for n in ('width', 'height', 'ncomp', 'hs', 'vs', 'mcus_x', 'mcus_y', 'restart_interval',
                               'first_interval', 'n_intervals')] + [
      ('qsel', C.c_uint8 * 4), ('dcsel', C.c_uint8 * 4), ('acsel', C.c_uint8 * 4), ('reserved', C.c_int32)]


class JpegHuff(C.Structure):
  _fields_ = [('bits', C.c_uint8 * 16), ('vals', C.c_uint8 * 256)]


class JpegTables(C.Structure):
  _fields_ = [('quant', (C.c_uint16 * 64) * 4), ('dc', JpegHuff * 2), ('ac', JpegHuff * 2)]


class JpegInterval(C.Structure):
  _fields_ = [('image', C.c_int32), ('first_mcu', C.c_int32), ('n_mcus', C.c_int32), ('rst', C.c_int32),
              ('byte_begin', C.c_int64), ('byte_end', C.c_int64)]


class JpegScan(C.Structure):
  _fields_ = [('image', C.c_int32), ('ncomp', C.c_int32), ('comp', C.c_uint8 * 4), ('ss', C.c_uint8), ('se', C.c_uint8),
              ('ah', C.c_uint8), ('al', C.c_uint8), ('huff', C.c_int32 * 3), ('restart_interval', C.c_int32),
              ('first_interval', C.c_int32), ('n_intervals', C.c_int32), ('byte_begin', C.c_int64), ('byte_end', C.c_int64)]


assert (C.sizeof(JpegDesc), C.sizeof(JpegHuff), C.sizeof(JpegTables), C.sizeof(JpegInterval)) == (96, 272, 1600, 32)
assert C.sizeof(JpegScan) == 56
JPEG_EBADCODE, JPEG_EOVERRUN, JPEG_ERESTART, JPEG_EDESC = 1, 2, 4, 8


class ConvDesc(C.Structure):
  _fields_ = [('N', C.c_int32), ('H', C.c_int32), ('W', C.c_int32), ('C', C.c_int32),
              ('K', C.c_int32), ('R', C.c_int32), ('S', C.c_int32),
              ('stride', C.c_int32), ('pad', C.c_int32),
              ('Ho', C.c_int32), ('Wo', C.c_int32),
              ('x_img_pitch', C.c_int64), ('x_row_pitch', C.c_int32), ('x_pix_pitch', C.c_int32),
              ('ldy', C.c_int32), ('out_f32', C.c_int32)]


class ModelCfg(C.Structure):
  _fields_ = [(n, C.c_int32) for n in (
      'resnet_size', 'resnet_version', 'num_classes', 'use_se_block', 'use_sk_block', 'use_resnet_d',
      'anti_alias_filter_size', 'anti_alias_type', 'bl_alpha', 'bl_beta', 'zero_gamma', 'no_downsample', 'pool_type',
      'embedding_size', 'dtype', 'mixup_type')] + [(n, C.c_float) for n in (
          'bn_momentum', 'bn_eps', 'loss_scale', 'label_smoothing', 'kd_temp', 'weight_decay', 'momentum')]


class PlanEntry(C.Structure):
  _fields_ = [(n, C.c_int32) for n in ('kind', 'N', 'H', 'W', 'C', 'K', 'R', 'S', 'stride', 'Ho', 'Wo', 'flags',
                                       'trainable', 'reserved')] + [
      ('param_offset', C.c_int64), ('param_elems', C.c_int64), ('name', C.c_char * 112)]


class PlanSummary(C.Structure):
  _fields_ = [('n_entries', C.c_int32), ('trainable_tensors', C.c_int32), ('trainable_elems', C.c_int64),
              ('forward_macs_per_image', C.c_int64), ('wgrad_workspace_bytes', C.c_int64)]


class Tuning(C.Structure):
  _fields_ = [(n, C.c_int32) for n in (
      'igemm_mode', 'igemm_tile', 'igemm_pfa', 'dgrad_parity', 'wgrad_halo', 'wgrad_big', 'wgrad_splits', 'bn_rows', 'igemm3',
      'gemm1', 'wgrad_ring', 'igemm8', 'dense_small')]


TUNING_ENV = {'ASM_IGEMM_MODE': 'igemm_mode', 'ASM_IGEMM_TILE': 'igemm_tile', 'ASM_IGEMM_PFA': 'igemm_pfa',
              'ASM_DGRAD_PARITY': 'dgrad_parity', 'ASM_WGRAD_HALO': 'wgrad_halo', 'ASM_WGRAD_BIG': 'wgrad_big',
              'ASM_WGRAD_SPLITS': 'wgrad_splits', 'ASM_BN_ROWS': 'bn_rows', 'ASM_IGEMM3': 'igemm3', 'ASM_GEMM1': 'gemm1',
              'ASM_WGRAD_RING': 'wgrad_ring', 'ASM_IGEMM8': 'igemm8', 'ASM_DENSE_SMALL': 'dense_small'}


def apply_env_tuning(lib) -> 'Tuning':
  t = Tuning()
  lib.asm_tuning_defaults(C.byref(t))
  for env, field in TUNING_ENV.items():
    v = os.environ.get(env)
    if v not in (None, ''):
      setattr(t, field, int(v))
  check_code = lib.asm_set_tuning(C.byref(t))
  if check_code != ASM_OK:
    raise ValueError('asm_set_tuning rejected the ASM_* overrides: %s' % (lib.asm_last_error() or b'').decode())
  return t


ASM_F32, ASM_BF16, ASM_F16 = 0, 1, 2
ASM_DGRAD_MASKED, ASM_DGRAD_POOLED, ASM_DGRAD_BNRED = 1, 2, 4
CONV_DGRAD_S2 = 5
CONV_DENSE = 6
ASM_AA_SCONV, ASM_AA_PROJ = 1, 2
POOL_TYPES = {'gap': 0, 'gem': 1, 'flatten': 2}
(PLAN_CONV, PLAN_BN, PLAN_DENSE, PLAN_MAXPOOL, PLAN_AVGPOOL, PLAN_BLURPOOL, PLAN_GAP, PLAN_GEM, PLAN_FLATTEN, PLAN_SK_GAP,
 PLAN_SK_SELECT, PLAN_SE_SCALE, PLAN_ADD) = range(13)

_P, _I, _F, _Z = C.c_void_p, C.c_int, C.c_float, C.c_size_t
_D = C.POINTER(ConvDesc)

SIGNATURES = {
    'asm_last_error': (C.c_char_p, []),
    'asm_abi_version': (_I, []),
    'asm_launch_count': (C.c_ulonglong, []),
    'asm_stream_join': (_I, [_P, _P]),
    'asm_memcpy_async': (_I, [_P, _P, _Z, _P]),
    'asm_allreduce_bucket': (_I, [_P, _Z, _I, _P, _P, _P]),
    'asm_tape_begin': (_I, []),
    'asm_tape_mark': (_I, []),
    'asm_tape_end': (_I, []),
    'asm_tape_info': (_I, [_I, C.POINTER(C.c_int64 * 6)]),
    'asm_tape_replay': (_I, [_I, _I]),
    'asm_tape_free': (_I, [_I]),
    'asm_tuning_defaults': (None, [C.POINTER(Tuning)]),
    'asm_set_tuning': (_I, [C.POINTER(Tuning)]),
    'asm_get_tuning': (None, [C.POINTER(Tuning)]),
    'asm_conv2d_fprop': (_I, [_D, _P, _P, _P, _P, _P]),
    'asm_conv2d_stats_blocks': (_I, [_D]),
    'asm_conv2d_dgrad': (_I, [_D, _P, _P, _P, _P, _P]),
    'asm_conv2d_dgrad_masked': (_I, [_D, _P, _P, _P, _P, _P, _P]),
    'asm_conv2d_dgrad_pooled': (_I, [_D, _P, _P, _P, _P, _P, _I, _I, _I, _I, _I, _I, _P, _P]),
    'asm_conv2d_dgrad_bnred_blocks': (_I, [_D]),
    'asm_conv2d_dgrad_bnred': (_I, [_D, _P, _P, _P, _P, _P, _P, _P, _P, _P]),
    'asm_conv2d_dgrad_kernel': (_I, [_D, _I]),
    'asm_conv2d_wgrad_workspace_bytes': (_Z, [_D]),
    'asm_conv2d_wgrad': (_I, [_D, _P, _P, _P, _P, _Z, _P]),
    'asm_filter_transpose': (_I, [_P, _P, _I, _I, _I, _I, _I, _P]),
    'asm_filter_transpose_batched': (_I, [_P, _P, _P, _I, C.c_longlong, _P]),
    'asm_filter_transpose_tiled': (_I, [_P, _P, _P, _I, _I, _P]),
    'asm_stem_pack_filter': (_I, [_P, _P, _I, _I, _P]),
    'asm_stem_unpack_grad': (_I, [_P, _P, _I, _I, _P]),
    'asm_stem_pad_input': (_I, [_P, _I, _P, _I, _I, _I, _P]),
    'asm_bn_stats_blocks': (_I, [_I, _I]),
    'asm_bn_stats': (_I, [_P, _I, _I, _P, _P]),
    'asm_bn_partials_compact': (_I, [_P, _I, _I, _P, _I, _P]),
    'asm_bn_finalize': (_I, [_P, _I, _I, _I, _P, _P, _F, _F, _P, _P, _P, _P, _P, _P, _P]),
    'asm_bn_infer_coeffs': (_I, [_I, _P, _P, _P, _P, _F, _P, _P, _P]),
    'asm_bn_apply': (_I, [_P, _P, _I, _I, _P, _P, _P, _I, _I, _I, _I, _P, _P]),
    'asm_bn_bwd_reduce': (_I, [_P, _P, _P, _I, _I, _I, _P, _P, _P, _P]),
    'asm_bn_bwd_finalize': (_I, [_P, _I, _I, _I, _P, _P, _P, _P, _P, _P, _P, _P, _P]),
    'asm_bn_bwd_finalize_raw': (_I, [_P, _I, _I, _I, _P, _P, _P, _P, _P, _P, _P, _P, _P]),
    'asm_bn_bwd_apply': (_I, [_P, _P, _P, _I, _I, _I, _P, _P, _P, _P, _P, _P]),
    'asm_maxpool3x3s2_fwd': (_I, [_P, _P, _P, _I, _I, _I, _I, _P]),
    'asm_maxpool3x3s2_bwd': (_I, [_P, _P, _P, _I, _I, _I, _I, _P]),
    'asm_avgpool_fwd': (_I, [_P, _P, _I, _I, _I, _I, _I, _I, _I, _I, _I, _I, _P]),
    'asm_avgpool_bwd': (_I, [_P, _P, _I, _I, _I, _I, _I, _I, _I, _I, _I, _I, _P, _P]),
    'asm_upsample2x_bwd': (_I, [_P, _P, _I, _I, _I, _I, _P]),
    'asm_upsample2x_bwd_masked': (_I, [_P, _P, _P, _I, _I, _I, _I, _P]),
    'asm_blurpool_fwd': (_I, [_P, _P, _I, _I, _I, _I, _I, _I, _P]),
    'asm_blurpool_bwd': (_I, [_P, _P, _I, _I, _I, _I, _I, _I, _P]),
    'asm_gap_fwd': (_I, [_P, _P, _I, _I, _I, _P]),
    'asm_gap_bwd': (_I, [_P, _P, _I, _I, _I, _P]),
    'asm_sk_gap': (_I, [_P, _P, _I, _I, _I, _P]),
    'asm_sk_select_fwd': (_I, [_P, _P, _P, _I, _I, _I, _P]),
    'asm_sk_select_bwd_att': (_I, [_P, _P, _P, _P, _I, _I, _I, _P]),
    'asm_sk_select_bwd_f': (_I, [_P, _P, _P, _P, _I, _I, _I, _P]),
    'asm_sk_gap_bn': (_I, [_P, _P, _P, _P, _I, _I, _I, _P]),
    'asm_sk_select_bn_fwd': (_I, [_P, _P, _P, _P, _P, _I, _I, _I, _P]),
    'asm_sk_select_bn_bwd_att': (_I, [_P, _P, _P, _P, _P, _P, _I, _I, _I, _P]),
    'asm_sk_bn_bwd_blocks': (_I, [_I, _I, _I]),
    'asm_sk_bn_bwd_reduce': (_I, [_P, _P, _P, _P, _P, _P, _P, _P, _I, _I, _I, _P, _P]),
    'asm_sk_bn_bwd_apply': (_I, [_P, _P, _P, _P, _P, _P, _P, _P, _P, _P, _I, _I, _I, _P]),
    'asm_sk_gap_bn_stats': (_I, [_P, _P, _P, _P, _P, _P, _P, _I, _I, _I, _P]),
    'asm_sk_select_bn_bwd_att_stats': (_I, [_P, _P, _P, _P, _P, _P, _P, _P, _P, _I, _I, _I, _P]),
    'asm_sk_bn_bwd_finalize': (_I, [_P, _P, _P, _P, _I, _I, _I, _P, _P, _P, _P, _P, _P, _P, _P, _P]),
    'asm_se_scale_fwd': (_I, [_P, _P, _P, _I, _I, _I, _P]),
    'asm_se_scale_bwd_e': (_I, [_P, _P, _P, _P, _I, _I, _I, _P]),
    'asm_se_scale_bwd_x': (_I, [_P, _P, _P, _P, _I, _I, _I, _P]),
    'asm_relu_fwd': (_I, [_P, _P, _Z, _P]),
    'asm_relu_bwd': (_I, [_P, _P, _P, _Z, _P]),
    'asm_add_bf16': (_I, [_P, _P, _P, _Z, _P]),
    'asm_mask_apply': (_I, [_P, _P, _P, _Z, _P]),
    'asm_bias_add_f32': (_I, [_P, _P, _I, _I, _I, _P]),
    'asm_bias_grad_bf16': (_I, [_P, _I, _I, _I, _P, _P]),
    'asm_cast_f32_to_bf16': (_I, [_P, _P, _Z, _P]),
    'asm_cast_bf16_to_f32': (_I, [_P, _P, _Z, _P]),
    'asm_softmax_ce': (_I, [_P, _I, _P, _P, _I, _I, _F, _F, _F, _P, _P, _I, _P]),
    'asm_onehot': (_I, [_P, _P, _I, _I, _P]),
    'asm_softmax_rows': (_I, [_P, _P, _I, _I, _F, _P]),
    'asm_mean_f32': (_I, [_P, _I, _P, _P]),
    'asm_mixup_meansub': (_I, [_P, _I, _I, _I, _I, _I, _P, _P, _P, _P]),
    'asm_mixup_labels': (_I, [_P, _I, _I, _I, _P, _P, _P, _P]),
    'asm_sigmoid_ce': (_I, [_P, _I, _P, _I, _I, _F, _P, _P, _P, _I, _P]),
    'asm_gem_fwd': (_I, [_P, _P, _P, _I, _I, _I, _F, _P]),
    'asm_gem_bwd': (_I, [_P, _P, _P, _P, _I, _I, _I, _F, _P]),
    'asm_dropblock_mask': (_I, [_P, _F, _I, _I, _I, _I, _P, _P, _P]),
    'asm_dropblock_mask_dev': (_I, [_P, _P, _I, _I, _I, _I, _P, _P, _P]),
    'asm_dropblock_apply': (_I, [_P, _P, _P, _P, _I, _P, _I, _I, _P]),
    'asm_eval_rows': (_I, [_P, _I, _P, _I, _I, _P, _P, _P, _P, _P]),
    'asm_eval_accumulate': (_I, [_P, _P, _P, _I, _P, _P]),
    'asm_embed_sqnorm': (_I, [_P, _I, _I, _I, _P, _P]),
    'asm_retrieval_topk_workspace_bytes': (_Z, [_I, _I, _I]),
    'asm_retrieval_topk': (_I, [_P, _I, _P, _I, _P, _P, _I, _I, _I, _I, _I, _I, _P, _P, _P, _Z, _P]),
    'asm_topk_merge': (_I, [_P, _P, _I, _I, _I, _P, _P, _P]),
    'asm_retrieval_topk_wide_workspace_bytes': (_Z, [_I, _I, _I]),
    'asm_retrieval_topk_wide': (_I, [_P, _I, _P, _I, _P, _P, _I, _I, _I, _I, _I, _I, _P, _P, _P, _Z, _P]),
    'asm_topk_merge_wide': (_I, [_P, _P, _I, _I, _I, _P, _P, _P]),
    'asm_recall_accumulate': (_I, [_P, _I, _I, _P, _P, _I, _I, _P, _I, _P, _P]),
    'asm_sgd_momentum': (_I, [_P, _P, _P, _P, _Z, _F, _F, _F, _F, _P]),
    'asm_conv2d_fprop_bn': (_I, [_P, _P, _P, _P, _P, _P, _P, _I, _P]),
    'asm_bn_apply2': (_I, [_P, _P, _P, _I, _I, _P, _P, _P, _P, _I, _P, _P]),
    'asm_bn_bwd_reduce2': (_I, [_P, _P, _P, _P, _I, _I, _P, _P, _P, _P, _P, _P, _P]),
    'asm_bn_bwd_apply2': (_I, [_P, _P, _P, _P, _I, _I, _P, _P, _P, _P]),
    'asm_bn_small_max_rows': (_I, []),
    'asm_bn_small_fwd': (_I, [_P, _P, _I, _I, _P, _P, _F, _F, _P, _P, _P, _P, _I, _P, _P]),
    'asm_bn_small_bwd': (_I, [_P, _P, _P, _I, _I, _P, _P, _P, _P, _P, _P, _P]),
# ... 68 lines not shown
```

### assembled_cnn_amd/nn.py

```python
from __future__ import annotations

import math
from collections import OrderedDict
from typing import Callable, Dict, List, NamedTuple, Optional, Tuple

import numpy as np
import torch

from . import ops

BN_EPS = 1e-5


def dual_bn_on() -> bool:
  return ops.knob('ASM_BN_DUAL', '1') != '0'


def lazy_dz_on() -> bool:
  return ops.knob('ASM_LAZY_DZ', '1') != '0'


def defer_bn_on() -> bool:
  return ops.knob('ASM_BN_DEFER', '1') != '0'

# ... 175 lines not shown
  def _view(self, arena, name):
    sp = self.specs[name]
    return arena[sp.offset:sp.offset + sp.numel].view(sp.shape)

  def w(self, name):
    return self._view(self.w32, name)

  def g(self, name):
    return self._view(self.g32, name)

  def m(self, name):
    return self._view(self.m32, name)

  def wb(self, name):
    return self._view(self.w16, name)

  def st(self, name):
    shape, _, off = self.state_specs[name]
    n = int(np.prod(shape))
    return self.state[off:off + n].view(shape)

  def refresh_shadows(self):
    ops.cast_f32_to_bf16(self.w32, self.w16)
    self.refresh_derived()

  def alloc_wt(self, name, K, RS, Cn, ldk) -> dict:
    ws = dict(name=name, K=K, RS=RS, C=Cn, ldk=ldk, offset=-1)
    self.wt_specs.append(ws)
    return ws

  def wt_view(self, ws) -> torch.Tensor:
    n = ws['C'] * ws['RS'] * ws['ldk']
    return self.wt16[ws['offset']:ws['offset'] + n]

  def refresh_derived(self):
    if self.wt_specs:
      ops.filter_transpose_tiled(self.w16, self.wt16, self._wt_table, len(self.wt_specs), self._wt_tiles)
    for fn in self.derived:
      fn()

  def num_params(self) -> int:
    return sum(sp.numel for sp in self.specs.values())


def variance_scaling_init(shape_krsc):
  k, r, s, c = shape_krsc
  std = math.sqrt(1.0 / (r * s * c)) / .87962566103423978

  def init(rng):
    out = rng.standard_normal(size=shape_krsc)
    bad = np.abs(out) > 2.0
    while bad.any():
      out[bad] = rng.standard_normal(size=int(bad.sum()))
      bad = np.abs(out) > 2.0
    return out * std
  return init


def glorot_uniform_init(shape_kc):
  k, c = shape_kc
  limit = math.sqrt(6.0 / (k + c))
  return lambda rng: rng.uniform(-limit, limit, size=shape_kc)


def const_init(shape, value):
  return lambda rng: np.full(shape, value, dtype=np.float32)


class SavedBN(NamedTuple):
  y: torch.Tensor
  M: int
  C: int
  gamma: torch.Tensor
  mean: torch.Tensor
  invstd: torch.Tensor
  bn: "BatchNorm"
  scale: torch.Tensor
  shift: torch.Tensor


class RedCtx(NamedTuple):
  y: torch.Tensor
  mask: Optional[torch.Tensor]


class Var(object):
  __slots__ = ('_data', 'shape', '_grad', 'grad_mask', 'grad_owned', 'needs_grad', 'deferred', 'bn_ctx', 'red_ctx', 'red',
               'pre_dy', 'pool_grad')

  def __init__(self, data, shape=None, needs_grad=True):
    self._data = data
    self.shape = tuple(data.shape) if data is not None else tuple(shape)
    self.needs_grad = needs_grad
    self._grad = self.grad_mask = self.pool_grad = self.red = self.pre_dy = None
    self.grad_owned = False
    self.deferred = self.bn_ctx = self.red_ctx = None

  @property
  def data(self):
    if self.bn_pending():
      s = self.deferred
      self._data = ops.bn_apply(s.y, s.M, s.C, s.scale, s.shift, None, 0, False)
    return self._data

  def bn_pending(self) -> bool:
    return self._data is None and self.deferred is not None

  @data.setter
  def data(self, t):
    self._data = t

  @property
  def grad(self):
    if self.grad_mask is not None:
      self.set_grad(ops.mask_apply(self._grad, self.grad_mask), True)
    if self.pool_grad is not None:
      pg, self.pool_grad = self.pool_grad, None
      self._add_scattered(*pg)
    return self._grad

  @grad.setter
  def grad(self, g):
    self.set_grad(g, False)

  def set_grad(self, g, owned: bool, red_part=None):
    self._grad, self.grad_mask, self.grad_owned = g, None, owned
    self.red = (red_part, g) if red_part is not None else None

  def add_grad(self, g, owned: bool, mask=None):
    self.red = None
    if mask is not None:
      if self._grad is None:
        self._grad, self.grad_mask, self.grad_owned = g, mask, False
        return
      g, owned = ops.mask_apply(g, mask), True
    cur = self.grad
    if cur is None:
      self.set_grad(g, owned)
    elif self.grad_owned:
      ops.add_bf16(cur, g, out=cur)
    else:
      self.set_grad(ops.add_bf16(cur, g), True)

  def add_pooled_grad(self, dp, k, stride, pad, count_valid, keep_pooled: bool):
    self.red = None
    if keep_pooled and self.pool_grad is None:
      self.pool_grad = (dp, k, stride, pad, count_valid)
    else:
      self.grad
      self._add_scattered(dp, k, stride, pad, count_valid)

  def _add_scattered(self, dp, k, stride, pad, count_valid):
    self.red = None
    if self._grad is None:
      self._grad = ops.avgpool_bwd(dp, self.shape, k, stride, pad, count_valid)
    elif self.grad_owned:
      ops.avgpool_bwd(dp, self.shape, k, stride, pad, count_valid, addend=self._grad)
    else:
      self._grad = ops.add_bf16(self._grad, ops.avgpool_bwd(dp, self.shape, k, stride, pad, count_valid))
    self.grad_owned = True

  def take_masked_grad(self):
    if self.pool_grad is not None:
      self.grad
    return self._grad, self.grad_mask

  def take_pool_grad(self, d):
    if self.pool_grad is None or not ops.dgrad_pool_ok(d):
      return None
    pg, self.pool_grad = self.pool_grad, None
    return pg

  def take_red(self, g, relu_mask):
    red, self.red = self.red, None
    ok = red is not None and red[1] is g and self.red_ctx is not None and self.red_ctx.mask is relu_mask
    return red[0] if ok else None

  def park_dy(self, dy):
    self.pre_dy = dy

  def take_dy(self):
    dy, self.pre_dy = self.pre_dy, None
    return dy

  def no_grad_yet(self) -> bool:
    return self._grad is None and self.pre_dy is None

  def held(self):
    return self._grad, self.grad_mask, self.pre_dy, self.pool_grad


def accum_grad(v: Var, g: torch.Tensor, owned: bool, mask: Optional[torch.Tensor] = None):
  if v.needs_grad:
    v.add_grad(g, owned, mask)


class Ctx(object):

  def __init__(self, arena: ParamArena, training: bool, dry: bool, bn_momentum: float, device,
               record_tape: bool, layers: Optional[list] = None):
    self.arena = arena
    self.layers = layers if layers is not None else []
    self._cursor = 0
    self.dlogits = None
    self.uniforms = None
    self.db_static = None
    self.rng = None
    self.training = training
    self.dry = dry
    self.bn_momentum = bn_momentum
    self.device = device
    self.tape: Optional[List[Callable[[], None]]] = [] if (record_tape and not dry) else None
    self.taps: "OrderedDict[str, torch.Tensor]" = OrderedDict()
    self._scope: List[str] = []
    self._counters: Dict[Tuple[str, str], int] = {}

  def next_uniform(self, shape):
    if self.uniforms is not None:
      u = next(self.uniforms)
      if tuple(u.shape) != tuple(shape):
        raise ValueError('dropblock uniform has shape %s, expected %s' % (tuple(u.shape), tuple(shape)))
      return u.contiguous()
    return torch.rand(shape, generator=self.rng, device=self.device, dtype=torch.float32)

  def layer(self, factory):
    if self.dry:
      obj = factory()
      self.layers.append(obj)
      return obj
    obj = self.layers[self._cursor]
    self._cursor += 1
    return obj

  def unique(self, base: str) -> str:
    key = ('/'.join(self._scope), base)
    n = self._counters.get(key, 0)
    self._counters[key] = n + 1
    return base if n == 0 else '%s_%d' % (base, n)

  def push_scope(self, default_name: str):
    self._scope.append(self.unique(default_name))

  def pop_scope(self):
    self._scope.pop()

  def full_name(self, layer: str, var: str) -> str:
    return '/'.join(['resnet_model'] + self._scope + [layer, var])

  def record(self, fn: Callable[[], None]):
    if self.tape is not None:
      self.tape.append(fn)

  def tap(self, name: str, v: Var):
    if not self.dry:
      self.taps[name] = v.data

  def backward(self):
    for fn in reversed(self.tape):
      fn()
# ... 27 lines not shown
        self._wts = ctx.arena.alloc_wt(self.name, cout, k * k, cin, self.kpad)

  def _refresh(self):
    a = self.arena
    dev = a.w32.device
    if self.stem:
      if self._wpack is None:
        self._wpack = torch.empty((self.cout, self.k, 1, self.stem_len), dtype=torch.bfloat16, device=dev)
      ops.stem_pack_filter(a.w(self.name), self._wpack, self.cout, self.k)

  def desc(self, N, H, W, stride, out_f32=False, ldy=0):
    if self.stem:
      Hp, Wp = H + 6, W + 6
      return ops.make_conv_desc(N, Hp, Wp, self.stem_len, self.cout, self.k, 1, 2, pad=0,
                                Ho=ops.out_size(H, self.k, 2), Wo=ops.out_size(W, self.k, 2),
                                img_pitch=Hp * Wp * 4, row_pitch=Wp * 4, pix_pitch=4, ldy=ldy, out_f32=out_f32)
    return ops.make_conv_desc(N, H, W, self.cin, self.cout, self.k, self.k, stride, ldy=ldy, out_f32=out_f32)

  def weight(self):
    return self._wpack if self.stem else self.arena.wb(self.name)

  def _stem_view(self, x: torch.Tensor) -> torch.Tensor:
    off = 3 - (self.k - 1) // 2
    if off == 0:
      return x
    Wp = x.shape[2]
    return x.view(-1)[(off * Wp + off) * 4:]

  def fprop(self, d, x: torch.Tensor, want_stats: bool):
    if self.stem:
      x = self._stem_view(x)
    return ops.conv_fprop(d, x, self.weight(), want_stats)

  def fprop_bn(self, d, x: torch.Tensor, scale, shift, residual, relu):
    if self.stem:
      x = self._stem_view(x)
    return ops.conv_fprop_bn(d, x, self.weight(), scale, shift, residual, relu)

  def _wgrad(self, d, x: torch.Tensor, dy: torch.Tensor):
    a = self.arena
    if self.stem:
      dwp = torch.empty((self.cout, self.k, self.stem_len), dtype=torch.float32, device=x.device)
      ops.conv_wgrad(d, self._stem_view(x), dy, dwp)
      ops.stem_unpack_grad(dwp, a.g(self.name), self.cout, self.k)
    else:
      ops.conv_wgrad(d, x, dy, a.g(self.name))

  def wgrad_streamed(self, d, x: torch.Tensor, dy: torch.Tensor):
    a = self.arena
    side = a.pick_side_stream()
    if side is not None:
      ops.stream_join(side, a.compute_stream or torch.cuda.current_stream())
      if self.stem or ops.timer_on():
        with torch.cuda.stream(side):
          self._wgrad(d, x, dy)
      else:
        ops.launch_on(side)
        try:
          self._wgrad(d, x, dy)
        finally:
          ops.launch_on(None)
      x.record_stream(side)
      dy.record_stream(side)
    else:
      self._wgrad(d, x, dy)
    a.notify_grad(self.name)

  def backward(self, d, x: torch.Tensor, dy: torch.Tensor, need_dx: bool,
               addend: Optional[torch.Tensor] = None, addend_mask: Optional[torch.Tensor] = None, pool=None
               ) -> Optional[torch.Tensor]:
    return self.backward_red(d, x, dy, need_dx, addend, addend_mask, pool, None)[0]

  def backward_red(self, d, x: torch.Tensor, dy: torch.Tensor, need_dx: bool, addend=None, addend_mask=None, pool=None,
                   red_ctx=None):
    a = self.arena
    self.wgrad_streamed(d, x, dy)
    if self.stem or not need_dx:
      return None, None
    if addend_mask is not None and (d.stride != 1 or d.C % 8) and not ops.dgrad_s2_ok(d):
      addend, addend_mask = ops.mask_apply(addend, addend_mask), None
    dd = d
    if self.kpad != self.cout:
      dd = ops.make_conv_desc(d.N, d.H, d.W, d.C, self.kpad, d.R, d.S, d.stride, pad=d.pad, Ho=d.Ho, Wo=d.Wo)
    if red_ctx is not None and pool is None and ops.dgrad_bnred_ok(dd):
      return ops.conv_dgrad_bnred(dd, dy, a.wt_view(self._wts), addend, addend_mask, red_ctx.y, red_ctx.mask)
    return ops.conv_dgrad(dd, dy, a.wt_view(self._wts), addend, addend_mask, pool), None


class BatchNorm(object):

  def __init__(self, ctx: Ctx, c: int, zero_gamma: bool = False, layer_name: Optional[str] = None):
    layer = ctx.unique('batch_normalization') if layer_name is None else layer_name
    self.c = c
    self.arena = ctx.arena
    self.gamma = ctx.full_name(layer, 'gamma')
    self.beta = ctx.full_name(layer, 'beta')
    self.mm = ctx.full_name(layer, 'moving_mean')
    self.mv = ctx.full_name(layer, 'moving_variance')
    ctx.arena.register(self.gamma, (c,), False, const_init((c,), 0.0 if zero_gamma else 1.0))
    ctx.arena.register(self.beta, (c,), False, const_init((c,), 0.0))
    ctx.arena.register_state(self.mm, (c,), 0.0)
    ctx.arena.register_state(self.mv, (c,), 1.0)


class ConvBnForm(NamedTuple):
  stats: str
  fold: bool
  apply: str
  want_mask: bool
  save_bn: bool
  offer_red: bool


def conv_bn_form(ctx: Ctx, conv: ConvKernel, d, M: int, relu: bool, residual: Optional[Var], rm: int,
                 tap_pre: Optional[str]) -> ConvBnForm:
  taped, Cn = ctx.tape is not None, conv.cout
  small = ctx.training and residual is None and d.Ho * d.Wo == 1 and not conv.stem and ops.bn_small_ok(M)
  stats = 'small' if small else 'batch' if ctx.training else 'moving'
  fold = not ctx.training and tap_pre is None and not taped and rm in (0, 1) and Cn % 8 == 0
  linear = ctx.training and not small and not relu and residual is None
  if small:
    apply = 'none'
  elif (residual is not None and rm == 1 and ctx.training and residual.bn_pending()
        and residual.deferred.M == M and residual.deferred.C == Cn):
    apply = 'dual'
  elif linear and tap_pre is None and Cn % 8 == 0 and defer_bn_on():
    apply = 'defer'
  else:
    apply = 'own'
  offer_red = (taped and ctx.training and apply in ('dual', 'own') and Cn % 8 == 0
               and not (residual is not None and residual.bn_ctx is not None and dual_bn_on()))
  return ConvBnForm(stats, fold, apply, taped and relu, taped and linear, offer_red)


def _with_mask(applied, want_mask: bool):
  return applied if want_mask else (applied, None)


def conv_bn(ctx: Ctx, x: Var, conv: ConvKernel, bn: BatchNorm, stride: int, relu: bool,
            residual: Optional[Var] = None, res_mode: int = 0, tap_pre: Optional[str] = None) -> Var:
  if conv.stem:
    N, Hp, Wp, _ = x.shape
    H, W = Hp - 6, Wp - 6
  else:
    N, H, W, _ = x.shape
  d = conv.desc(N, H, W, stride)
  out_shape = (N, d.Ho, d.Wo, conv.cout)
  if ctx.dry:
    return Var(None, out_shape)
  a = ctx.arena
  M = N * d.Ho * d.Wo
  Cn = conv.cout
  gamma, beta = a.w(bn.gamma), a.w(bn.beta)
  rm = res_mode if residual is not None else 0
  form = conv_bn_form(ctx, conv, d, M, relu, residual, rm, tap_pre)
  small = form.stats == 'small'
  res_t = residual.data if (residual is not None and form.apply != 'dual') else None
  out_t = mask_t = mean = invstd = None
  if small:
    y, _ = conv.fprop(d, x.data, False)
    out_t, mask_t, mean, invstd = ops.bn_small_fwd(y, M, Cn, gamma, beta, BN_EPS, ctx.bn_momentum, a.st(bn.mm),
                                                   a.st(bn.mv), relu, want_mask=form.want_mask)
  elif form.stats == 'batch':
    y, part = conv.fprop(d, x.data, True)
    mean, invstd, scale, shift = ops.bn_finalize(part, M, Cn, gamma, beta, BN_EPS, ctx.bn_momentum,
                                                 a.st(bn.mm), a.st(bn.mv))
  elif form.fold:
    scale, shift = ops.bn_infer_coeffs(Cn, gamma, beta, a.st(bn.mm), a.st(bn.mv), BN_EPS)
    return Var(conv.fprop_bn(d, x.data, scale, shift, res_t if rm == 1 else None, relu))
  else:
    y, _ = conv.fprop(d, x.data, False)
    scale, shift = ops.bn_infer_coeffs(Cn, gamma, beta, a.st(bn.mm), a.st(bn.mv), BN_EPS)
  if tap_pre is not None:
    ctx.taps[tap_pre] = y
  if form.apply == 'dual':
    sc = residual.deferred
    out_t, mask_t = _with_mask(ops.bn_apply_dual(y, sc.y, M, Cn, scale, shift, sc.scale, sc.shift, relu,
                                                 want_mask=form.want_mask), form.want_mask)
  elif form.apply == 'own':
    out_t, mask_t = _with_mask(ops.bn_apply(y, M, Cn, scale, shift, res_t, rm, relu, d.Ho, d.Wo, want_mask=form.want_mask),
                               form.want_mask)
  out = Var(out_t, out_shape)
  if form.apply == 'defer' or form.save_bn:
    saved = SavedBN(y, M, Cn, gamma, mean, invstd, bn, scale, shift)
    if form.apply == 'defer':
      out.deferred = saved
    if form.save_bn:
      out.bn_ctx = saved
  if form.offer_red:
    out.red_ctx = RedCtx(y, mask_t)

  if ctx.tape is not None:
    x_t = x.data

    def bwd():
      dy = out.take_dy()
      if dy is not None:
        a.notify_grad(bn.gamma)
        conv_input_grad(conv, d, x, x_t, dy, want_red=False)
        return
      dout, in_mask = out.take_masked_grad()
      if dout is None:
        raise RuntimeError('conv_bn backward: no gradient reached this layer')
      bmask, brelu = mask_t, relu
      if in_mask is not None:
        if relu or small or residual is not None:
          dout = out.grad
        else:
          bmask, brelu = in_mask, True
      sc = residual.bn_ctx if (residual is not None and rm == 1) else None
      if residual is None:
        route = 'none'
      elif not relu:
        route = 'dout'
      elif not (lazy_dz_on() and (residual.needs_grad if rm == 1 else rm == 2)):
        route = 'dz'
      elif sc is not None and residual.no_grad_yet() and sc.M == M and sc.C == Cn and dual_bn_on():
        route = 'dual'
      else:
        route = 'lazy'
      dz = None
      if small:
        dy = ops.bn_small_bwd(dout, y, bmask, M, Cn, gamma, mean, invstd, a.g(bn.gamma), a.g(bn.beta))
      elif route == 'dual':
        dy, dy_sc = ops.bn_bwd_dual(dout, y, sc.y, mask_t, M, Cn,
                                    (gamma, mean, invstd, a.g(bn.gamma), a.g(bn.beta)),
                                    (sc.gamma, sc.mean, sc.invstd, a.g(sc.bn.gamma), a.g(sc.bn.beta)))
        residual.park_dy(dy_sc)
      else:
        dy, dz = ops.bn_bwd(dout, y, bmask, brelu, M, Cn, gamma, mean, invstd, a.g(bn.gamma), a.g(bn.beta),
                            route == 'dz', raw_part=out.take_red(dout, bmask))
      a.notify_grad(bn.gamma)
      if route in ('lazy', 'dz', 'dout'):
        g, g_mask, owned = (dout, mask_t, False) if route == 'lazy' else (dz, None, True) if route == 'dz' else (dout, None, False)
        if rm == 2:
          g, g_mask, owned = ops.upsample2x_bwd(g, g_mask), None, True
        accum_grad(residual, g, owned, mask=g_mask)
      conv_input_grad(conv, d, x, x_t, dy)
      out.grad = None
    bwd.relu_mask = mask_t
    ctx.record(bwd)
  return out


def conv_input_grad(conv: ConvKernel, d, x: Var, x_t: torch.Tensor, dy: torch.Tensor, want_red: bool = True):
  pool = x.take_pool_grad(d) if (conv.kpad == conv.cout and x.needs_grad) else None
  xg, xmask = x.take_masked_grad()
  dx, part = conv.backward_red(d, x_t, dy, x.needs_grad, xg, xmask, pool, x.red_ctx if want_red else None)
  if dx is not None:
    x.set_grad(dx, True, part)


def conv_plain(ctx: Ctx, x: Var, conv: ConvKernel, out_f32: bool, ldy: int = 0):
  N, H, W, _ = x.shape
  d = conv.desc(N, H, W, 1, out_f32=out_f32, ldy=ldy)
  if ctx.dry:
    return None, None, (N, d.Ho, d.Wo, ldy if ldy else conv.cout)
  y, _ = conv.fprop(d, x.data, False)
  x_t = x.data

  def bwd(dy: torch.Tensor):
    dd = ops.make_conv_desc(d.N, d.H, d.W, d.C, d.K, d.R, d.S, d.stride, pad=d.pad, Ho=d.Ho, Wo=d.Wo,
                            ldy=ldy if (ldy and ldy != conv.cout) else 0)
    conv_input_grad(conv, dd, x, x_t, dy, want_red=False)
  return y, bwd, tuple(y.shape)


class SKUnit(object):

  def __init__(self, ctx: Ctx, cin: int, filters: int, r: int = 2, L: int = 32):
    self.filters = filters
    self.conv = ConvKernel(ctx, 3, cin, filters * 2)
    self.bn = BatchNorm(ctx, filters * 2)
    self.d = max(int(filters / r), L)
    ctx.push_scope('sk_block')
    self.fc1 = ConvKernel(ctx, 1, filters, self.d, layer_name='sk_fc_1')
    self.bn1 = BatchNorm(ctx, self.d)
    self.fc2 = ConvKernel(ctx, 1, self.d, filters * 2, layer_name='sk_fc_2')
    ctx.pop_scope()

  def __call__(self, ctx: Ctx, x: Var, stride: int) -> Var:
    if ctx.training and not ctx.dry and 2 * self.filters <= 2048 and ops.knob('ASM_SK_FUSED', '1') != '0':
      return self._call_fused(ctx, x, stride)
    F_ = self.filters
    f = conv_bn(ctx, x, self.conv, self.bn, stride, relu=True)
    N, H, W, _ = f.shape
    if ctx.dry:
      return Var(None, (N, H, W, F_))
    s = Var(ops.sk_gap(f.data, F_))
    z = conv_bn(ctx, s, self.fc1, self.bn1, 1, relu=True)
    att, fc2_bwd, _ = conv_plain(ctx, z, self.fc2, out_f32=True)
    v_t = ops.sk_select_fwd(f.data, att, F_)
    v = Var(v_t)
    if ctx.tape is not None:
      bwd_z = ctx.tape.pop()
      bwd_f = ctx.tape.pop()
      f_t = f.data

      def bwd():
        dv = v.grad
        datt = ops.sk_select_bwd_att(f_t, dv, att, F_)
        fc2_bwd(datt)
        bwd_z()
        df = ops.sk_select_bwd_f(dv, att, s.grad, F_)
        s.grad = None
        accum_grad(f, df, True)
        bwd_f()
        v.grad = None
      ctx.record(bwd)
    return v
# ... 289 lines not shown
```

### assembled_cnn_amd/ops.py

```python
from __future__ import annotations

import ctypes as C
import os
from typing import Optional, Tuple

import torch

from . import lib as _lib
from .lib import ConvDesc, check

_L = None
_IS_DOUBLE = False


def set_library(obj, is_double: bool = False):
  global _L, _IS_DOUBLE
  _L = obj
  _IS_DOUBLE = is_double


def L():
  global _L
  if _L is None:
    _L = _lib.load()
# ... 147 lines not shown
      return None
    e0 = torch.cuda.Event(enable_timing=True)
    e1 = torch.cuda.Event(enable_timing=True)
    e0.record()
    self.events.setdefault(k, []).append((e0, e1))
    return e1

  def start_class(self, cls, work):
    e0 = torch.cuda.Event(enable_timing=True)
    e1 = torch.cuda.Event(enable_timing=True)
    e0.record()
    self.class_events.setdefault(cls, []).append((e0, e1, float(work)))
    return e1

  def summary(self):
    return {k: (len(v), sum(a.elapsed_time(b) for a, b in v)) for k, v in self.events.items()}

  def class_summary(self):
    return {k: (len(v), sum(a.elapsed_time(b) for a, b, _ in v), sum(w for _, _, w in v))
            for k, v in self.class_events.items()}


_TIMER: Optional[ConvTimer] = None


def set_conv_timer(t: Optional[ConvTimer]):
  global _TIMER
  _TIMER = t


def timer_on() -> bool:
  return _TIMER is not None


def _bn_ev(nbytes):
  return _TIMER.start_class('bn', nbytes) if (_TIMER is not None and _TIMER.classes) else None


def conv_fprop(d: ConvDesc, x: torch.Tensor, w: torch.Tensor, want_stats: bool = False
               ) -> Tuple[torch.Tensor, Optional[torch.Tensor]]:
  ldy = d.ldy if d.ldy else d.K
  y = empty((d.N, d.Ho, d.Wo, ldy), F32 if d.out_f32 else BF16, x)
  stats = None
  if want_stats:
    stats = empty((L().asm_conv2d_stats_blocks(C.byref(d)), 2, d.K), F32, x)
  ev = _TIMER.start('fprop', d) if _TIMER is not None else None
  check(L().asm_conv2d_fprop(C.byref(d), _ptr(x), _ptr(w), _ptr(y), _ptr(stats), _stream()), 'conv2d_fprop')
  if ev is not None:
    ev.record()
  return y, stats


def conv_fprop_bn(d: ConvDesc, x: torch.Tensor, w: torch.Tensor, scale, shift, residual=None, relu=False):
  y = empty((d.N, d.Ho, d.Wo, d.K), BF16, x)
  ev = _TIMER.start('fprop', d) if _TIMER is not None else None
  check(L().asm_conv2d_fprop_bn(C.byref(d), _ptr(x), _ptr(w), _ptr(y), _ptr(scale), _ptr(shift), _ptr(residual),
                                1 if relu else 0, _stream()), 'conv2d_fprop_bn')
  if ev is not None:
    ev.record()
  return y


def dgrad_kernel(d: ConvDesc, variant: int = 0) -> int:
  query = getattr(L(), 'asm_conv2d_dgrad_kernel', None)
  if query is None:
    return _lib.ASM_ENOTSUP
  return query(C.byref(d), variant)


def dgrad_pool_ok(d: ConvDesc) -> bool:
  return (knob('ASM_POOL_FUSE', '1') != '0' and d.K % 32 == 0
          and dgrad_kernel(d, _lib.ASM_DGRAD_POOLED) >= 0)


def dgrad_s2_ok(d: ConvDesc) -> bool:
  return dgrad_kernel(d) == _lib.CONV_DGRAD_S2


def dgrad_bnred_ok(d: ConvDesc) -> bool:
  mode = knob('ASM_BN_RED', '1')
  if mode == '0' or (mode == '1x1' and d.R != 1):
    return False
  return dgrad_kernel(d, _lib.ASM_DGRAD_BNRED) >= 0


def conv_dgrad_bnred(d: ConvDesc, dy: torch.Tensor, wt: torch.Tensor, addend, addend_mask, bn_y: torch.Tensor, bn_mask):
  dx = empty((d.N, d.H, d.W, d.C), BF16, dy)
  blocks = L().asm_conv2d_dgrad_bnred_blocks(C.byref(d))
  part = empty((blocks, 2, d.C), F32, dy)
  ev = _TIMER.start('dgrad', d) if _TIMER is not None else None
  check(L().asm_conv2d_dgrad_bnred(C.byref(d), _ptr(dy), _ptr(wt), _ptr(addend), _ptr(addend_mask), _ptr(bn_y), _ptr(bn_mask),
                                   _ptr(part), _ptr(dx), _stream()), 'conv2d_dgrad_bnred')
  if ev is not None:
    ev.record()
  return dx, part


def conv_dgrad(d: ConvDesc, dy: torch.Tensor, wt: torch.Tensor, addend: Optional[torch.Tensor] = None,
               addend_mask: Optional[torch.Tensor] = None, pool=None) -> torch.Tensor:
  dx = empty((d.N, d.H, d.W, d.C), BF16, dy)
  ev = None
  if _TIMER is not None:
    ev = _TIMER.start('dgrad+add' if (addend is not None and getattr(_TIMER, 'split_addend', False)) else 'dgrad', d)
  if pool is not None:
    pdy, pk, pst, ppad, pcv = pool
    check(L().asm_conv2d_dgrad_pooled(C.byref(d), _ptr(dy), _ptr(wt), _ptr(addend), _ptr(addend_mask), _ptr(pdy), pk, pst,
                                      ppad, pdy.shape[1], pdy.shape[2], 1 if pcv else 0, _ptr(dx), _stream()),
          'conv2d_dgrad_pooled')
    if ev is not None:
      ev.record()
    return dx
  if addend_mask is not None:
    check(L().asm_conv2d_dgrad_masked(C.byref(d), _ptr(dy), _ptr(wt), _ptr(addend), _ptr(addend_mask), _ptr(dx),
                                      _stream()), 'conv2d_dgrad_masked')
  else:
    check(L().asm_conv2d_dgrad(C.byref(d), _ptr(dy), _ptr(wt), _ptr(addend), _ptr(dx), _stream()), 'conv2d_dgrad')
  if ev is not None:
    ev.record()
  return dx


_ws_cache = {}
_ws_retired = []


def _workspace(nbytes: int, like: torch.Tensor) -> Optional[torch.Tensor]:
  if nbytes == 0:
    return None
  key = (str(like.device), _stream())
  buf = _ws_cache.get(key)
  if buf is None or buf.numel() < nbytes:
    if buf is not None:
      _ws_retired.append(buf)
    buf = torch.empty((nbytes,), dtype=torch.uint8, device=like.device)
    _ws_cache[key] = buf
  return buf


def conv_wgrad(d: ConvDesc, x: torch.Tensor, dy: torch.Tensor, dw: torch.Tensor):
  need = L().asm_conv2d_wgrad_workspace_bytes(C.byref(d))
  ws = _workspace(need, x)
  ev = _TIMER.start('wgrad', d) if _TIMER is not None else None
  check(L().asm_conv2d_wgrad(C.byref(d), _ptr(x), _ptr(dy), _ptr(dw), _ptr(ws), need, _stream()), 'conv2d_wgrad')
  if ev is not None:
    ev.record()


def filter_transpose(w: torch.Tensor, wt: torch.Tensor, K, R, S, Cin, ldk=0):
  check(L().asm_filter_transpose(_ptr(w), _ptr(wt), K, R, S, Cin, ldk, _stream()), 'filter_transpose')


def filter_transpose_batched(w_arena, wt_arena, table, nlayers, total):
  check(L().asm_filter_transpose_batched(_ptr(w_arena), _ptr(wt_arena), _ptr(table), nlayers, total, _stream()),
        'filter_transpose_batched')


def filter_transpose_tiled(w_arena, wt_arena, table, nlayers, total_tiles):
  check(L().asm_filter_transpose_tiled(_ptr(w_arena), _ptr(wt_arena), _ptr(table), nlayers, total_tiles, _stream()),
        'filter_transpose_tiled')


def stem_pack_filter(w32: torch.Tensor, wp: torch.Tensor, K: int, ksize: int):
  check(L().asm_stem_pack_filter(_ptr(w32), _ptr(wp), K, ksize, _stream()), 'stem_pack_filter')


def stem_unpack_grad(dwp: torch.Tensor, dw: torch.Tensor, K: int, ksize: int):
# ... 19 lines not shown
  check(L().asm_bn_stats(_ptr(x2d), M, Cn, _ptr(part), _stream()), 'bn_stats')
  return part


def _compact(part: torch.Tensor, Cn: int) -> torch.Tensor:
  blocks = part.shape[0]
  if blocks <= 1024:
    return part
  per = -(-blocks // 32)
  groups = -(-blocks // per)
  out = empty((groups, 2, Cn), F32, part)
  check(L().asm_bn_partials_compact(_ptr(part), blocks, Cn, _ptr(out), groups, _stream()), 'bn_partials_compact')
  return out


def bn_finalize(part, M, Cn, gamma, beta, eps, momentum, mm, mv):
  ev = _bn_ev(part.numel() * 4.0)
  part = _compact(part, Cn)
  co = empty((4, Cn), F32, part)
  check(L().asm_bn_finalize(_ptr(part), part.shape[0], M, Cn, _ptr(gamma), _ptr(beta), eps, momentum,
                            _ptr(mm), _ptr(mv), _ptr(co[0]), _ptr(co[1]), _ptr(co[2]), _ptr(co[3]),
                            _stream()), 'bn_finalize')
  if ev is not None:
    ev.record()
  return co[0], co[1], co[2], co[3]


def bn_infer_coeffs(Cn, gamma, beta, mm, mv, eps):
  co = empty((2, Cn), F32, gamma)
  check(L().asm_bn_infer_coeffs(Cn, _ptr(gamma), _ptr(beta), _ptr(mm), _ptr(mv), eps, _ptr(co[0]), _ptr(co[1]),
                                _stream()), 'bn_infer_coeffs')
  return co[0], co[1]


def bn_apply(x, M, Cn, scale, shift, residual=None, res_mode=0, relu=False, H=0, W=0, want_mask=False):
  y = torch.empty_like(x)
  mask = empty((M, Cn // 8), torch.uint8, x) if (want_mask and relu) else None
  ev = _bn_ev(M * Cn * (4.0 + (2.0 if res_mode == 1 else 0.5 if res_mode == 2 else 0.0) + (0.125 if mask is not None else 0.0)))
  check(L().asm_bn_apply(_ptr(x), _ptr(y), M, Cn, _ptr(scale), _ptr(shift), _ptr(residual), res_mode,
                         1 if relu else 0, H, W, _ptr(mask), _stream()), 'bn_apply')
  if ev is not None:
    ev.record()
  return (y, mask) if want_mask else y


def _bn_bwd_coeffs(part, M, Cn, gamma, mean, invstd, dgamma, dbeta, co, raw=False):
  part = _compact(part, Cn)
  fin, what = (L().asm_bn_bwd_finalize_raw, 'bn_bwd_finalize_raw') if raw else (L().asm_bn_bwd_finalize, 'bn_bwd_finalize')
  check(fin(_ptr(part), part.shape[0], M, Cn, _ptr(gamma), _ptr(mean), _ptr(invstd), _ptr(dgamma), _ptr(dbeta),
            _ptr(co[0]), _ptr(co[1]), _ptr(co[2]), _stream()), what)


def bn_bwd(dy, x, yout, relu, M, Cn, gamma, mean, invstd, dgamma, dbeta, want_dz, raw_part=None):
  rk = 0 if not relu else (2 if yout.dtype == torch.uint8 else 1)
  red_bytes = 0.0 if raw_part is not None else (4.0 + (0.125 if rk == 2 else 2.0 if rk == 1 else 0.0))
  ev = _bn_ev(M * Cn * (red_bytes + 4.0 + 2.0 + (2.0 if want_dz else 0.0) + (0.125 if rk == 2 else 2.0 if rk == 1 else 0.0)))
  co = empty((3, Cn), F32, dy)
  part = raw_part
  if part is None:
    part = empty((L().asm_bn_stats_blocks(M, Cn), 2, Cn), F32, dy)
    check(L().asm_bn_bwd_reduce(_ptr(dy), _ptr(x), _ptr(yout if relu else None), rk, M, Cn,
                                _ptr(mean), _ptr(invstd), _ptr(part), _stream()), 'bn_bwd_reduce')
  _bn_bwd_coeffs(part, M, Cn, gamma, mean, invstd, dgamma, dbeta, co, raw=raw_part is not None)
  dx = torch.empty_like(x)
  dz = torch.empty_like(x) if want_dz else None
  check(L().asm_bn_bwd_apply(_ptr(dy), _ptr(x), _ptr(yout if relu else None), rk, M, Cn,
                             _ptr(co[0]), _ptr(co[1]), _ptr(co[2]), _ptr(dx), _ptr(dz), _stream()), 'bn_bwd_apply')
  if ev is not None:
    ev.record()
  return dx, dz


def bn_apply_dual(xa, xb, M, Cn, scale_a, shift_a, scale_b, shift_b, relu, want_mask=False):
  y = torch.empty_like(xa)
  mask = empty((M, Cn // 8), torch.uint8, xa) if (want_mask and relu) else None
  ev = _bn_ev(M * Cn * (6.0 + (0.125 if mask is not None else 0.0)))
  check(L().asm_bn_apply2(_ptr(xa), _ptr(xb), _ptr(y), M, Cn, _ptr(scale_a), _ptr(shift_a), _ptr(scale_b), _ptr(shift_b),
                          1 if relu else 0, _ptr(mask), _stream()), 'bn_apply2')
  if ev is not None:
    ev.record()
  return (y, mask) if want_mask else y


def bn_bwd_dual(dy, xa, xb, mask, M, Cn, bn_a, bn_b):
  ev = _bn_ev(M * Cn * (2 * 6.0 + 4.0 + 2 * 0.125))
  blocks = L().asm_bn_stats_blocks(M, Cn)
  pa, pb = empty((blocks, 2, Cn), F32, dy), empty((blocks, 2, Cn), F32, dy)
  check(L().asm_bn_bwd_reduce2(_ptr(dy), _ptr(xa), _ptr(xb), _ptr(mask), M, Cn, _ptr(bn_a[1]), _ptr(bn_a[2]),
                               _ptr(bn_b[1]), _ptr(bn_b[2]), _ptr(pa), _ptr(pb), _stream()), 'bn_bwd_reduce2')
  co = empty((6, Cn), F32, dy)
  for i, (part, (gamma, mean, invstd, dgamma, dbeta)) in enumerate(((pa, bn_a), (pb, bn_b))):
    _bn_bwd_coeffs(part, M, Cn, gamma, mean, invstd, dgamma, dbeta, co[3 * i:3 * i + 3])
  dxa, dxb = torch.empty_like(xa), torch.empty_like(xb)
  check(L().asm_bn_bwd_apply2(_ptr(dy), _ptr(xa), _ptr(xb), _ptr(mask), M, Cn, _ptr(co), _ptr(dxa), _ptr(dxb), _stream()),
        'bn_bwd_apply2')
  if ev is not None:
    ev.record()
  return dxa, dxb


_SMALL_BN_ROWS = None


def bn_small_ok(M: int) -> bool:
  global _SMALL_BN_ROWS
  if _SMALL_BN_ROWS is None:
    _SMALL_BN_ROWS = int(L().asm_bn_small_max_rows())
  return M <= _SMALL_BN_ROWS


def bn_small_fwd(x, M, Cn, gamma, beta, eps, momentum, mm, mv, relu, want_mask):
  y = torch.empty_like(x)
  co = empty((2, Cn), F32, x)
  mask = empty((M, Cn // 8), torch.uint8, x) if (want_mask and relu) else None
  check(L().asm_bn_small_fwd(_ptr(x), _ptr(y), M, Cn, _ptr(gamma), _ptr(beta), eps, momentum, _ptr(mm), _ptr(mv),
                             _ptr(co[0]), _ptr(co[1]), 1 if relu else 0, _ptr(mask), _stream()), 'bn_small_fwd')
  return y, mask, co[0], co[1]


def bn_small_bwd(dy, x, mask, M, Cn, gamma, mean, invstd, dgamma, dbeta):
  dx = torch.empty_like(x)
  check(L().asm_bn_small_bwd(_ptr(dy), _ptr(x), _ptr(mask), M, Cn, _ptr(gamma), _ptr(mean), _ptr(invstd),
                             _ptr(dgamma), _ptr(dbeta), _ptr(dx), _stream()), 'bn_small_bwd')
  return dx


def maxpool3x3s2_fwd(x):
  N, H, W, Cn = x.shape
  Ho, Wo = (H + 1) // 2, (W + 1) // 2
  y = empty((N, Ho, Wo, Cn), BF16, x)
  am = empty((N, Ho, Wo, Cn), torch.uint8, x)
  check(L().asm_maxpool3x3s2_fwd(_ptr(x), _ptr(y), _ptr(am), N, H, W, Cn, _stream()), 'maxpool_fwd')
  return y, am


def maxpool3x3s2_bwd(dy, am, in_shape):
  N, H, W, Cn = in_shape
  dx = empty(in_shape, BF16, dy)
  check(L().asm_maxpool3x3s2_bwd(_ptr(dy), _ptr(am), _ptr(dx), N, H, W, Cn, _stream()), 'maxpool_bwd')
  return dx


def avgpool_fwd(x, k, stride, pad, Ho, Wo, count_valid):
  N, H, W, Cn = x.shape
  y = empty((N, Ho, Wo, Cn), BF16, x)
  check(L().asm_avgpool_fwd(_ptr(x), _ptr(y), N, H, W, Cn, k, stride, pad, Ho, Wo, 1 if count_valid else 0,
                            _stream()), 'avgpool_fwd')
  return y


def avgpool_bwd(dy, in_shape, k, stride, pad, count_valid, addend=None):
  N, H, W, Cn = in_shape
  dx = addend if addend is not None else empty(in_shape, BF16, dy)
  check(L().asm_avgpool_bwd(_ptr(dy), _ptr(dx), N, H, W, Cn, k, stride, pad, dy.shape[1], dy.shape[2],
                            1 if count_valid else 0, _ptr(addend), _stream()), 'avgpool_bwd')
  return dx


def upsample2x_bwd(dy, mask=None):
  N, H, W, Cn = dy.shape
  dx = empty((N, H // 2, W // 2, Cn), BF16, dy)
  if mask is not None:
    check(L().asm_upsample2x_bwd_masked(_ptr(dy), _ptr(mask), _ptr(dx), N, H // 2, W // 2, Cn, _stream()),
          'upsample2x_bwd_masked')
  else:
    check(L().asm_upsample2x_bwd(_ptr(dy), _ptr(dx), N, H // 2, W // 2, Cn, _stream()), 'upsample2x_bwd')
  return dx


def blur_out_size(n, k, stride):
  return (n + 2 * ((k - 1) // 2) - k) // stride + 1


def blurpool_fwd(x, k, stride):
  N, H, W, Cn = x.shape
# ... 465 lines not shown
```

### include/asm_hip.h

```cpp
#ifndef ASM_HIP_H_
#define ASM_HIP_H_

#include <stddef.h>
#include <stdint.h>

#ifdef __cplusplus
extern "C" {
#endif

#define ASM_OK 0
#define ASM_EINVAL (-1)
#define ASM_ENOTSUP (-2)
#define ASM_EHIP (-3)

#define ASM_ABI_VERSION 11

const char* asm_last_error(void);
int asm_abi_version(void);
unsigned long long asm_launch_count(void);

int asm_stream_join(void* dst_stream, void* src_stream);
int asm_memcpy_async(void* dst, const void* src, size_t bytes, void* stream);

int asm_allreduce_bucket(void* buf, size_t count, int dtype, void* nccl_comm, void* comm_stream, void* producer_stream);
int asm_tape_begin(void);
int asm_tape_mark(void);
int asm_tape_end(void);
int asm_tape_info(int tape, int64_t info[6]);
int asm_tape_replay(int tape, int segment);
int asm_tape_free(int tape);

typedef struct asm_tuning {
  int32_t igemm_mode;
  int32_t igemm_tile;
  int32_t igemm_pfa;
  int32_t dgrad_parity;
  int32_t wgrad_halo;
  int32_t wgrad_big;
  int32_t wgrad_splits;
  int32_t bn_rows;
  int32_t igemm3;
  int32_t gemm1;
  int32_t wgrad_ring;
  int32_t igemm8;
  int32_t dense_small;
} asm_tuning;
void asm_tuning_defaults(asm_tuning* t);
int asm_set_tuning(const asm_tuning* t);
void asm_get_tuning(asm_tuning* t);

typedef struct asm_conv_desc {
  int32_t N, H, W, C;
  int32_t K, R, S;
  int32_t stride, pad;
  int32_t Ho, Wo;
  int64_t x_img_pitch;
  int32_t x_row_pitch;
  int32_t x_pix_pitch;
  int32_t ldy;
  int32_t out_f32;
} asm_conv_desc;

int asm_conv2d_fprop(const asm_conv_desc* d, const void* x, const void* w, void* y,
                     float* stats_partial, void* stream);
int asm_conv2d_stats_blocks(const asm_conv_desc* d);

int asm_conv2d_fprop_bn(const asm_conv_desc* d, const void* x, const void* w, void* y, const float* scale,
                        const float* shift, const void* residual, int relu, void* stream);

int asm_conv2d_dgrad(const asm_conv_desc* d, const void* dy, const void* wt, const void* addend, void* dx,
                     void* stream);

int asm_conv2d_dgrad_masked(const asm_conv_desc* d, const void* dy, const void* wt, const void* addend,
                            const uint8_t* addend_mask, void* dx, void* stream);
int asm_conv2d_dgrad_pooled(const asm_conv_desc* d, const void* dy, const void* wt, const void* addend,
                            const uint8_t* addend_mask, const void* pool_dy, int pool_k, int pool_stride, int pool_pad,
                            int pool_Ho, int pool_Wo, int count_valid, void* dx, void* stream);

int asm_conv2d_dgrad_bnred_blocks(const asm_conv_desc* d);
int asm_conv2d_dgrad_bnred(const asm_conv_desc* d, const void* dy, const void* wt, const void* addend,
                           const uint8_t* addend_mask, const void* bn_y, const uint8_t* bn_relu_mask, float* partial,
                           void* dx, void* stream);

#define ASM_DGRAD_MASKED 1
#define ASM_DGRAD_POOLED 2
#define ASM_DGRAD_BNRED 4
int asm_conv2d_dgrad_kernel(const asm_conv_desc* d, int variant);

size_t asm_conv2d_wgrad_workspace_bytes(const asm_conv_desc* d);
int asm_conv2d_wgrad(const asm_conv_desc* d, const void* x, const void* dy, float* dw,
                     void* workspace, size_t workspace_bytes, void* stream);

int asm_filter_transpose(const void* w_krsc, void* w_crsk, int K, int R, int S, int C, int ldk, void* stream);

int asm_filter_transpose_batched(const void* w_arena, void* wt_arena, const int32_t* table, int nlayers,
                                 long long total_elems, void* stream);
int asm_filter_transpose_tiled(const void* w_arena, void* wt_arena, const int32_t* table, int nlayers,
                               int total_tiles, void* stream);

int asm_stem_pack_filter(const float* w_krsc3, void* w_packed, int K, int ksize, void* stream);
int asm_stem_unpack_grad(const float* dw_packed, float* dw_krsc3, int K, int ksize, void* stream);
int asm_stem_pad_input(const void* x, int x_is_f32, void* xp, int N, int H, int W, void* stream);

int asm_bn_stats_blocks(int M, int C);
int asm_bn_stats(const void* x, int M, int C, float* stats_partial, void* stream);
int asm_bn_partials_compact(const float* partial, int blocks, int C, float* out, int groups, void* stream);
int asm_bn_finalize(const float* stats_partial, int blocks, int M, int C, const float* gamma,
                    const float* beta, float eps, float momentum, float* moving_mean,
                    float* moving_var, float* mean, float* invstd, float* scale, float* shift,
                    void* stream);
int asm_bn_infer_coeffs(int C, const float* gamma, const float* beta, const float* moving_mean,
                        const float* moving_var, float eps, float* scale, float* shift, void* stream);
int asm_bn_apply(const void* x, void* y, int M, int C, const float* scale, const float* shift,
                 const void* residual, int res_mode, int relu, int H, int W, uint8_t* relu_mask_out,
                 void* stream);
int asm_bn_bwd_reduce(const void* dy, const void* x, const void* yout, int relu, int M, int C,
                      const float* mean, const float* invstd, float* partial, void* stream);
int asm_bn_bwd_finalize(const float* partial, int blocks, int M, int C, const float* gamma,
                        const float* mean, const float* invstd, float* dgamma, float* dbeta,
                        float* coefA, float* coefB, float* coefC, void* stream);
int asm_bn_bwd_finalize_raw(const float* partial, int blocks, int M, int C, const float* gamma,
                            const float* mean, const float* invstd, float* dgamma, float* dbeta,
                            float* coefA, float* coefB, float* coefC, void* stream);
int asm_bn_bwd_apply(const void* dy, const void* x, const void* yout, int relu, int M, int C,
                     const float* coefA, const float* coefB, const float* coefC, void* dx,
                     void* dz_out, void* stream);

int asm_bn_apply2(const void* xa, const void* xb, void* y, int M, int C, const float* scale_a, const float* shift_a,
                  const float* scale_b, const float* shift_b, int relu, uint8_t* relu_mask_out, void* stream);
int asm_bn_bwd_reduce2(const void* dy, const void* xa, const void* xb, const uint8_t* relu_mask, int M, int C,
                       const float* mean_a, const float* invstd_a, const float* mean_b, const float* invstd_b,
                       float* partial_a, float* partial_b, void* stream);
int asm_bn_bwd_apply2(const void* dy, const void* xa, const void* xb, const uint8_t* relu_mask, int M, int C,
                      const float* coef6, void* dxa, void* dxb, void* stream);

int asm_bn_small_max_rows(void);
int asm_bn_small_fwd(const void* x, void* y, int M, int C, const float* gamma, const float* beta, float eps,
                     float momentum, float* moving_mean, float* moving_var, float* mean, float* invstd, int relu,
                     uint8_t* relu_mask_out, void* stream);
int asm_bn_small_bwd(const void* dy, const void* x, const uint8_t* relu_mask, int M, int C, const float* gamma,
                     const float* mean, const float* invstd, float* dgamma, float* dbeta, void* dx, void* stream);

int asm_dense_small(const void* p, int ldp, const void* q, int ldq, int M, int N, int K, void* out, int ldo,
                    int out_f32, const void* addend, void* stream);
int asm_dense_small_wgrad(const void* x, int ldx, const void* dy, int ldy, int M, int Cin, int Cout, float* dw, int ldw,
                          void* stream);

int asm_maxpool3x3s2_fwd(const void* x, void* y, uint8_t* argmax, int N, int H, int W, int C, void* stream);
int asm_maxpool3x3s2_bwd(const void* dy, const uint8_t* argmax, void* dx, int N, int H, int W, int C, void* stream);
int asm_avgpool_fwd(const void* x, void* y, int N, int H, int W, int C, int k, int stride, int pad,
                    int Ho, int Wo, int count_valid, void* stream);
int asm_avgpool_bwd(const void* dy, void* dx, int N, int H, int W, int C, int k, int stride, int pad,
                    int Ho, int Wo, int count_valid, const void* addend, void* stream);
int asm_upsample2x_bwd(const void* dy, void* dx, int N, int Hs, int Ws, int C, void* stream);
int asm_upsample2x_bwd_masked(const void* dy, const uint8_t* relu_mask, void* dx, int N, int Hs, int Ws, int C,
                              void* stream);
int asm_blurpool_fwd(const void* x, void* y, int N, int H, int W, int C, int k, int stride, void* stream);
int asm_blurpool_bwd(const void* dy, void* dx, int N, int H, int W, int C, int k, int stride, void* stream);
int asm_gap_fwd(const void* x, void* y, int N, int HW, int C, void* stream);
int asm_gap_bwd(const void* dy, void* dx, int N, int HW, int C, void* stream);

int asm_sk_gap(const void* f, void* s, int N, int HW, int F, void* stream);
int asm_sk_select_fwd(const void* f, const float* att, void* v, int N, int HW, int F, void* stream);
int asm_sk_select_bwd_att(const void* f, const void* dv, const float* att, void* datt, int N, int HW, int F, void* stream);
int asm_sk_select_bwd_f(const void* dv, const float* att, const void* ds, void* df, int N, int HW, int F, void* stream);
int asm_sk_gap_bn(const void* y, const float* scale, const float* shift, void* s, int N, int HW, int F, void* stream);
int asm_sk_select_bn_fwd(const void* y, const float* scale, const float* shift, const float* att, void* v, int N,
                         int HW, int F, void* stream);
int asm_sk_select_bn_bwd_att(const void* y, const float* scale, const float* shift, const void* dv, const float* att,
// ... 224 lines not shown
```

Baseline: 10830 images/sec.

## Fuse dual batch-norm and pooled-gradient reductions into 1x1 dgrad epilogues

Extends the 1x1 dgrad GEMM epilogues so they can accumulate the batch-norm backward sums for two batch norms at once (main branch plus shortcut), and can also do so when an average-pool backward is folded in. The separate bn_bwd_reduce2 pass over dy and both activations is then skipped, and its partials come from the conv epilogue instead. This removes one full memory pass per affected block. The cost is a heavier epilogue with extra loads of the second activation, more template variants, and a forced BK=64 tile for some narrow-channel layers.

```diff
diff --git a/assembled_cnn_amd/csrc/conv_gemm1.hip b/assembled_cnn_amd/csrc/conv_gemm1.hip
--- a/assembled_cnn_amd/csrc/conv_gemm1.hip
+++ b/assembled_cnn_amd/csrc/conv_gemm1.hip
@@ -33,7 +33,7 @@
   static_assert(LDS <= 160 * 1024, "lds");
 };
 
-template <int BM, int BN, int BK, int WGM, int WGN, bool STATS, int NS, bool PFA, bool POOL, bool BNRED = false>
+template <int BM, int BN, int BK, int WGM, int WGN, bool STATS, int NS, bool PFA, bool POOL, int BNRED = 0>
 __global__ __launch_bounds__(64 * WGM * WGN) void igemm1_kernel(IGemmArgs p) {
   using C = Cfg<BM, BN, BK, WGM, WGN, false, STATS>;
   using C1 = Cfg1<BM, BN, BK, WGM, WGN, NS>;
@@ -175,7 +175,7 @@
   igemm_epilogue<C, BM, BN, WTM, WTN, TM, TN, false, STATS, PFA, POOL, false, BNRED>(p, acc, smem, tile_m, tile_n, tid, wm, wn, l31, lhi);
 }
 
-template <int BM, int BN, int BK, int WGM, int WGN, bool STATS, int NS, bool PFA, bool POOL, bool BNRED = false>
+template <int BM, int BN, int BK, int WGM, int WGN, bool STATS, int NS, bool PFA, bool POOL, int BNRED = 0>
 int launch1_one(const IGemmArgs& a, hipStream_t st) {
   using C1 = Cfg1<BM, BN, BK, WGM, WGN, NS>;
   auto kern = igemm1_kernel<BM, BN, BK, WGM, WGN, STATS, NS, PFA, POOL, BNRED>;
@@ -190,7 +190,10 @@
 template <int BM, int BN, int BK, int WGM, int WGN, int NS>
 int launch1(const ConvLaunch& L, const IGemmArgs& a, hipStream_t st) {
   switch (L.epi) {
-    case EPI_BNRED: return launch1_one<BM, BN, BK, WGM, WGN, true, NS, false, false, true>(a, st);
+    case EPI_BNRED: return launch1_one<BM, BN, BK, WGM, WGN, true, NS, false, false, 1>(a, st);
+    case EPI_BNRED2: return launch1_one<BM, BN, BK, WGM, WGN, true, NS, false, false, 2>(a, st);
+    case EPI_POOL_BNRED: return launch1_one<BM, BN, BK, WGM, WGN, true, NS, false, true, 1>(a, st);
+    case EPI_POOL_BNRED2: return launch1_one<BM, BN, BK, WGM, WGN, true, NS, false, true, 2>(a, st);
     case EPI_STATS: return launch1_one<BM, BN, BK, WGM, WGN, true, NS, false, false>(a, st);
     case EPI_POOL: return launch1_one<BM, BN, BK, WGM, WGN, false, NS, false, true>(a, st);
     case EPI_PFA: return launch1_one<BM, BN, BK, WGM, WGN, false, NS, true, false>(a, st);
diff --git a/assembled_cnn_amd/csrc/conv_igemm.hip b/assembled_cnn_amd/csrc/conv_igemm.hip
--- a/assembled_cnn_amd/csrc/conv_igemm.hip
+++ b/assembled_cnn_amd/csrc/conv_igemm.hip
@@ -178,7 +178,7 @@
 };
 
 template <int BM, int BN, int BK, int WGM, int WGN, bool OUT_F32, bool STATS, int R, int S, int NS, bool PFA = false, bool POOL = false,
-          int SCHED = 0, bool BNRED = false>
+          int SCHED = 0, int BNRED = 0>
 __global__ __launch_bounds__(64 * WGM * WGN) void igemm2_kernel(IGemmArgs p) {
   using C = Cfg<BM, BN, BK, WGM, WGN, OUT_F32, STATS>;
   using C2 = Cfg2<BM, BN, BK, WGM, WGN, OUT_F32, STATS, NS>;
@@ -752,7 +752,7 @@
 }
 
 template <int BM, int BN, int BK, int WGM, int WGN, bool OUT_F32, bool STATS, int R, int S, int NS = 2, bool PFA = false, bool POOL = false,
-          int SCHED = 0, bool BNRED = false>
+          int SCHED = 0, int BNRED = 0>
 int launch2_one(const IGemmArgs& a, hipStream_t st) {
   using C = Cfg2<BM, BN, BK, WGM, WGN, OUT_F32, STATS, NS>;
   constexpr int NTHR = 64 * WGM * WGN;
@@ -770,7 +770,8 @@
 
 constexpr unsigned igemm2_variants(int R, int S, int BM, int BN, int BK) {
   if (R == 1 && S == 1)
-    return epi_bit(EPI_F32) | epi_bit(EPI_BNRED) | epi_bit(EPI_STATS) | epi_bit(EPI_POOL) | epi_bit(EPI_PFA) | epi_bit(EPI_PLAIN);
+    return epi_bit(EPI_F32) | epi_bit(EPI_BNRED) | epi_bit(EPI_STATS) | epi_bit(EPI_POOL) | epi_bit(EPI_PFA) | epi_bit(EPI_PLAIN) |
+           (BM == 128 ? epi_bit(EPI_POOL_BNRED) | epi_bit(EPI_BNRED2) | epi_bit(EPI_POOL_BNRED2) : 0u);
   if (R == 3 && S == 3) return epi_bit(EPI_STATS) | epi_bit(EPI_PFA) | epi_bit(EPI_PLAIN);
   if ((R == 1 && S == 2) || (R == 2 && S == 1) || (R == 2 && S == 2)) return epi_bit(EPI_PLAIN);
   if ((R == 7 || R == 3) && S == 1 && BK == 32 && BM == 128 && BN <= 64) return epi_bit(EPI_STATS) | epi_bit(EPI_PLAIN);
@@ -783,7 +784,13 @@
   if constexpr ((has >> EPI_F32) & 1)
     if (L.epi == EPI_F32) return launch2_one<BM, BN, BK, WGM, WGN, true, false, R, S>(a, st);
   if constexpr ((has >> EPI_BNRED) & 1)
-    if (L.epi == EPI_BNRED) return launch2_one<BM, BN, BK, WGM, WGN, false, true, R, S, 2, false, false, 0, true>(a, st);
+    if (L.epi == EPI_BNRED) return launch2_one<BM, BN, BK, WGM, WGN, false, true, R, S, 2, false, false, 0, 1>(a, st);
+  if constexpr ((has >> EPI_BNRED2) & 1)
+    if (L.epi == EPI_BNRED2) return launch2_one<BM, BN, BK, WGM, WGN, false, true, R, S, 2, false, false, 0, 2>(a, st);
+  if constexpr ((has >> EPI_POOL_BNRED) & 1)
+    if (L.epi == EPI_POOL_BNRED) return launch2_one<BM, BN, BK, WGM, WGN, false, true, R, S, 2, false, true, 0, 1>(a, st);
+  if constexpr ((has >> EPI_POOL_BNRED2) & 1)
+    if (L.epi == EPI_POOL_BNRED2) return launch2_one<BM, BN, BK, WGM, WGN, false, true, R, S, 2, false, true, 0, 2>(a, st);
   if constexpr ((has >> EPI_STATS) & 1)
     if (L.epi == EPI_STATS) return launch2_one<BM, BN, BK, WGM, WGN, false, true, R, S>(a, st);
   if constexpr ((has >> EPI_POOL) & 1)
@@ -843,7 +850,7 @@
   return t.bk == 64 ? F<128, 128, 64, 2, 2>::run(L, a, st) : F<128, 128, 32, 2, 2>::run(L, a, st);
 }
 
-enum class ConvOut { bf16, f32, stats, bnred };
+enum class ConvOut { bf16, f32, stats, bnred, bnred2 };
 
 bool tile256(const IGemmArgs& a) {
   const int ftile = asm_tune().igemm_tile;
@@ -868,7 +875,9 @@
     case FAM_IGEMM2: return igemm2_variants(a.R, a.S, t.bm, t.bn, t.bk);
     case FAM_HALO: return epi_bit(EPI_STATS) | epi_bit(EPI_PLAIN);
     case FAM_DENSE: return epi_bit(EPI_F32) | epi_bit(EPI_PLAIN);
-    case FAM_GEMM1: return epi_bit(EPI_BNRED) | epi_bit(EPI_STATS) | epi_bit(EPI_POOL) | epi_bit(EPI_PFA) | epi_bit(EPI_PLAIN);
+    case FAM_GEMM1:
+      return epi_bit(EPI_BNRED) | epi_bit(EPI_STATS) | epi_bit(EPI_POOL) | epi_bit(EPI_PFA) | epi_bit(EPI_PLAIN) |
+             epi_bit(EPI_POOL_BNRED) | epi_bit(EPI_BNRED2) | epi_bit(EPI_POOL_BNRED2);
     default: return epi_bit(EPI_BNRED) | epi_bit(EPI_STATS) | epi_bit(EPI_PFA) | epi_bit(EPI_PLAIN);
   }
 }
@@ -883,7 +892,8 @@
   const int pfa_env = asm_tune().igemm_pfa;
   const bool pfa = (has & epi_bit(EPI_PFA)) && a.addend != nullptr && !a.y_strided &&
                    (pfa_env >= 0 ? pfa_env != 0 : (t.bm == 256 || L.n_blocks <= 1024));
-  const int want = out == ConvOut::f32 ? EPI_F32 : out == ConvOut::bnred ? EPI_BNRED : out == ConvOut::stats ? EPI_STATS
+  const int want = out == ConvOut::f32 ? EPI_F32 : out == ConvOut::bnred ? (a.pool_dy ? EPI_POOL_BNRED : EPI_BNRED)
+                   : out == ConvOut::bnred2 ? (a.pool_dy ? EPI_POOL_BNRED2 : EPI_BNRED2) : out == ConvOut::stats ? EPI_STATS
                    : a.pool_dy ? EPI_POOL : pfa ? EPI_PFA : EPI_PLAIN;
   L.epi = (has & epi_bit(want)) ? want : -1;
   if (family == FAM_IGEMM3) {
@@ -909,14 +919,16 @@
 
 ConvPlan plan_conv(const IGemmArgs& a, ConvOut out) {
   const asm_tuning& tu = asm_tune();
-  const bool f32 = out == ConvOut::f32, stats = out == ConvOut::stats || out == ConvOut::bnred;
+  const bool red = out == ConvOut::bnred || out == ConvOut::bnred2;
+  const bool f32 = out == ConvOut::f32, stats = out == ConvOut::stats || red;
   const bool k1 = a.R == 1 && a.S == 1;
-  const bool bnred3 = out == ConvOut::bnred && !k1;
+  const bool bnred3 = red && !k1;
   if (dense_covers(a, out)) return single(tiled(FAM_DENSE, ConvTile{32, 32, 16, 1, 1}, a, out, a.M, 0));
-  if (dense_shaped(a) && (a.pool_dy || out == ConvOut::bnred))
+  if (dense_shaped(a) && (a.pool_dy || red))
     return no_plan("conv dgrad: the fused input-gradient forms do not take a [N,1,1,C] layer");
-  if (a.pool_dy && (tu.igemm_mode != 0 || out != ConvOut::bf16 || !k1 || a.y_strided))
-    return no_plan("conv dgrad_pooled: only the 1x1 stride-1 igemm2 path folds an average-pool backward in");
+  if (out == ConvOut::bnred2 && !k1) return no_plan("conv dgrad: only the 1x1 kernels reduce the sums of two batch norms");
+  if (a.pool_dy && (tu.igemm_mode != 0 || (out != ConvOut::bf16 && !red) || !k1 || a.y_strided))
+    return no_plan("conv dgrad_pooled: only the 1x1 stride-1 igemm1 / igemm2 path folds an average-pool backward in");
   if (tu.igemm_mode == 0 && tu.igemm_tile == 0) {
     if (halo_covers(a, f32)) {
       if (bnred3) return no_plan("conv dgrad_bnred: no kernel with the batch-norm sums for this 3x3 layer");
@@ -958,7 +970,8 @@
     if (cov3 && (h3 == 2 || !big || to_igemm3)) return single(tiled(FAM_IGEMM3, t128, a, out, a.M, 0));
   }
   if (bnred3) return no_plan("conv dgrad_bnred: no kernel with the batch-norm sums for this 3x3 layer");
-  const ConvTile t = pick_tile(a);
+  ConvTile t = pick_tile(a);
+  if ((a.pool_dy || out == ConvOut::bnred2) && t.bm == 128 && t.bk == 32 && a.Ci > 32 && a.Ci < 64) t.bk = 64;
   if (tu.igemm_mode == 0) {
     const ConvLaunch L = tiled(FAM_IGEMM2, t, a, out, a.M, 0);
     if (L.epi >= 0 && (a.Ci % t.bk == 0 || a.Ci <= t.bk)) return single(L);
@@ -1071,6 +1084,8 @@
   const void* y;
   const uint8_t* mask;
   float* partial;
+  const void* y2;
+  float* partial2;
 };
 static int dgrad_impl(const asm_conv_desc* d, const void* dy, const void* wt, const void* addend,
                       const uint8_t* addend_mask, void* dx, void* stream, const PoolAdd* pool = nullptr,
@@ -1192,13 +1207,17 @@
   return dgrad_impl(d, dy, wt, addend, addend_mask, dx, stream, &pa);
 }
 
-static bool dgrad_bnred_covers(const asm_conv_desc* d) {
+static bool dgrad_bnred_covers(const asm_conv_desc* d, bool pooled = false, bool dual = false) {
   if (!d || d->C % 8 || d->K % 8 || d->stride != 1 || d->x_img_pitch || d->x_row_pitch || d->x_pix_pitch || d->out_f32) return false;
-  if (!(d->R == 1 && d->S == 1 && d->pad == 0) && !(d->R == 3 && d->S == 3 && d->pad == 1 && d->Ho == d->H && d->Wo == d->W))
-    return false;
-  const ConvPlan p = plan_conv(dgrad_args(d), ConvOut::bnred);
+  const bool k1 = d->R == 1 && d->S == 1 && d->pad == 0;
+  if (!k1 && (pooled || dual || !(d->R == 3 && d->S == 3 && d->pad == 1 && d->Ho == d->H && d->Wo == d->W))) return false;
+  alignas(16) static const unsigned char operand[16] = {};
+  IGemmArgs a = dgrad_args(d);
+  if (pooled) a.pool_dy = operand;
+  const ConvPlan p = plan_conv(a, dual ? ConvOut::bnred2 : ConvOut::bnred);
+  const int epi = dual ? (pooled ? EPI_POOL_BNRED2 : EPI_BNRED2) : (pooled ? EPI_POOL_BNRED : EPI_BNRED);
   for (int i = 0; i < p.n; ++i)
-    if (p.l[i].epi != EPI_BNRED) return false;
+    if (p.l[i].epi != epi) return false;
   return p.n > 0;
 }
 
@@ -1216,17 +1235,47 @@
   if (!dgrad_bnred_covers(d))
     ASM_FAIL(ASM_ENOTSUP, "conv dgrad_bnred: 1x1 stride-1 layers, and the 3x3 stride-1 layers of the igemm8 / igemm3 kernels, with "
              "C %% 8 == 0 only (%dx%d, stride %d, C %d)", d->R, d->S, d->stride, d->C);
-  const BnRed r = {bn_y, bn_relu_mask, partial};
+  const BnRed r = {bn_y, bn_relu_mask, partial, nullptr, nullptr};
   return dgrad_impl(d, dy, wt, addend, addend_mask, dx, stream, nullptr, &r);
+}
+
+extern "C" int asm_conv2d_dgrad_pooled_bnred_blocks(const asm_conv_desc* d, int variant) {
+  if (!d || (variant & ~(ASM_DGRAD_MASKED | ASM_DGRAD_POOLED | ASM_DGRAD_BNRED | ASM_DGRAD_BNRED2))) return ASM_EINVAL;
+  if (!dgrad_bnred_covers(d, variant & ASM_DGRAD_POOLED, variant & ASM_DGRAD_BNRED2)) return 0;
+  return cdiv(d->N * d->H * d->W, STATS_BM);
+}
+
+extern "C" int asm_conv2d_dgrad_pooled_bnred(const asm_conv_desc* d, const void* dy, const void* wt, const void* addend,
+                                             const uint8_t* addend_mask, const void* pool_dy, int pool_k, int pool_stride,
+                                             int pool_pad, int pool_Ho, int pool_Wo, int count_valid, const void* bn_y,
+                                             const void* bn_y2, const uint8_t* bn_relu_mask, float* partial, float* partial2,
+                                             void* dx, void* stream) {
+  ASM_REQUIRE(d && bn_y && partial, "conv dgrad_pooled_bnred: null pointer");
+  ASM_REQUIRE(!bn_y2 == !partial2, "conv dgrad_pooled_bnred: a second batch norm needs its y and its partials");
+  ASM_REQUIRE(!addend_mask || addend, "conv dgrad_pooled_bnred: a mask needs its addend");
+  if (!dgrad_bnred_covers(d, pool_dy != nullptr, bn_y2 != nullptr))
+    ASM_FAIL(ASM_ENOTSUP, "conv dgrad_pooled_bnred: not covered (%dx%d, stride %d, C %d, %s, %s): see "
+             "asm_conv2d_dgrad_pooled_bnred_blocks", d->R, d->S, d->stride, d->C, pool_dy ? "pooled" : "not pooled",
+             bn_y2 ? "two batch norms" : "one batch norm");
+  const BnRed r = {bn_y, bn_relu_mask, partial, bn_y2, partial2};
+  if (!pool_dy) return dgrad_impl(d, dy, wt, addend, addend_mask, dx, stream, nullptr, &r);
+  ASM_REQUIRE(pool_k >= 1 && (pool_stride == 1 || pool_stride == 2) && pool_pad >= 0 && pool_Ho > 0 && pool_Wo > 0,
+              "conv dgrad_pooled_bnred: bad pooling geometry");
+  if (pool_k > 2 * pool_stride || pool_k < pool_stride)
+    ASM_FAIL(ASM_ENOTSUP, "conv dgrad_pooled_bnred: window %d / stride %d puts a pixel in more than two windows per dimension",
+             pool_k, pool_stride);
+  const PoolAdd pa = {pool_dy, pool_k, pool_stride, pool_pad, pool_Ho, pool_Wo, count_valid ? 1 : 0};
+  return dgrad_impl(d, dy, wt, addend, addend_mask, dx, stream, &pa, &r);
 }
 
 extern "C" int asm_conv2d_dgrad_kernel(const asm_conv_desc* d, int variant) {
   if (int e = dgrad_check(d)) return e;
-  ASM_REQUIRE(!(variant & ~(ASM_DGRAD_MASKED | ASM_DGRAD_POOLED | ASM_DGRAD_BNRED)), "conv dgrad_kernel: bad variant %d", variant);
-  const bool pooled = variant & ASM_DGRAD_POOLED, bnred = variant & ASM_DGRAD_BNRED;
-  if (pooled && (bnred || d->R != 1 || d->S != 1 || d->stride != 1 || d->pad != 0))
-    ASM_FAIL(ASM_ENOTSUP, "conv dgrad_kernel: the pooled input gradient is a 1x1 stride-1 one without the batch-norm sums");
-  if (bnred && !dgrad_bnred_covers(d)) ASM_FAIL(ASM_ENOTSUP, "conv dgrad_kernel: no batch-norm sums for this layer");
+  ASM_REQUIRE(!(variant & ~(ASM_DGRAD_MASKED | ASM_DGRAD_POOLED | ASM_DGRAD_BNRED | ASM_DGRAD_BNRED2)),
+              "conv dgrad_kernel: bad variant %d", variant);
+  const bool pooled = variant & ASM_DGRAD_POOLED, dual = variant & ASM_DGRAD_BNRED2, bnred = dual || (variant & ASM_DGRAD_BNRED);
+  if (pooled && (d->R != 1 || d->S != 1 || d->stride != 1 || d->pad != 0))
+    ASM_FAIL(ASM_ENOTSUP, "conv dgrad_kernel: the pooled input gradient is a 1x1 stride-1 one");
+  if (bnred && !dgrad_bnred_covers(d, pooled, dual)) ASM_FAIL(ASM_ENOTSUP, "conv dgrad_kernel: no batch-norm sums for this layer");
   alignas(16) static const unsigned char operand[16] = {};
   IGemmArgs a = dgrad_args(d);
   if (variant & ASM_DGRAD_MASKED) {
@@ -1234,7 +1283,7 @@
     a.addend_mask = operand;
   }
   if (pooled) a.pool_dy = operand;
-  const DgradPlan p = plan_dgrad(d, a, bnred ? ConvOut::bnred : ConvOut::bf16, true);
+  const DgradPlan p = plan_dgrad(d, a, dual ? ConvOut::bnred2 : bnred ? ConvOut::bnred : ConvOut::bf16, true);
   if (p.form == DgradForm::s2) return FAM_DGRAD_S2;
   const ConvPlan& last = p.form == DgradForm::parity ? p.cp[p.nc - 1] : p.conv;
   if (last.n == 0) ASM_FAIL(ASM_ENOTSUP, "%s", last.why);
@@ -1249,6 +1298,7 @@
   a.x = dy; a.w = wt; a.y = dx; a.addend = addend; a.addend_mask = addend_mask;
   if (red) {
     a.stats = red->partial; a.red_y = red->y; a.red_mask = red->mask;
+    a.red_y2 = red->y2; a.stats2 = red->partial2;
   }
   if (pool) {
     a.pool_dy = pool->dy; a.pool_k = pool->k; a.pool_stride = pool->stride; a.pool_pad = pool->pad;
@@ -1256,7 +1306,7 @@
   }
   const bool aligned = ((reinterpret_cast<uintptr_t>(dy) | reinterpret_cast<uintptr_t>(wt) | reinterpret_cast<uintptr_t>(dx) |
                          reinterpret_cast<uintptr_t>(addend)) & 15) == 0;
-  const DgradPlan p = plan_dgrad(d, a, red ? ConvOut::bnred : ConvOut::bf16, aligned);
+  const DgradPlan p = plan_dgrad(d, a, !red ? ConvOut::bf16 : red->y2 ? ConvOut::bnred2 : ConvOut::bnred, aligned);
   const hipStream_t st = (hipStream_t)stream;
   switch (p.form) {
     case DgradForm::s2:
diff --git a/assembled_cnn_amd/csrc/igemm_common.h b/assembled_cnn_amd/csrc/igemm_common.h
--- a/assembled_cnn_amd/csrc/igemm_common.h
+++ b/assembled_cnn_amd/csrc/igemm_common.h
@@ -45,12 +45,14 @@
   const uint8_t* red_mask;
   const void* pool_dy;
   int pool_k, pool_stride, pool_pad, pool_Hp, pool_Wp, pool_cv, pool_H;
+  const void* red_y2;
+  float* stats2;
 };
 
 constexpr int STATS_BM = 128;
 
 enum ConvFamily { FAM_GENERAL = 0, FAM_GEMM1 = 1, FAM_IGEMM2 = 2, FAM_IGEMM3 = 3, FAM_HALO = 4, FAM_DGRAD_S2 = 5, FAM_DENSE = 6, FAM_IGEMM8 = 8 };
-enum ConvEpi { EPI_PLAIN, EPI_PFA, EPI_POOL, EPI_STATS, EPI_BNRED, EPI_F32 };
+enum ConvEpi { EPI_PLAIN, EPI_PFA, EPI_POOL, EPI_STATS, EPI_BNRED, EPI_F32, EPI_POOL_BNRED, EPI_BNRED2, EPI_POOL_BNRED2 };
 constexpr unsigned epi_bit(int e) { return 1u << e; }
 struct ConvTile {
   int bm, bn, bk, wgm, wgn;
@@ -103,7 +105,7 @@
 };
 
 template <class C, int BM, int BN, int WTM, int WTN, int TM, int TN, bool OUT_F32, bool STATS, bool PFA = false, bool POOL = false,
-          bool SPLIT8 = false, bool BNRED = false, int RPF = 1>
+          bool SPLIT8 = false, int BNRED = 0, int RPF = 1>
 __device__ __forceinline__ void igemm_epilogue(const IGemmArgs& p, f32x16 (&acc)[TN][TM], unsigned char* smem,
                                                int tile_m, int tile_n, int tid, int wm, int wn, int l31, int lhi,
                                                int patch_base = -1) {
@@ -234,30 +236,34 @@
     };
     if constexpr (POOL) pool_issue(0, pcur);
     constexpr int SG = STATS ? BM / STATS_BM : 1;
-    float s[SG][8], ss[SG][8];
+    float s[SG][8], ss[SG][8], ss2[SG][8];
 #pragma unroll
     for (int q = 0; q < SG; ++q)
 #pragma unroll
-      for (int e = 0; e < 8; ++e) s[q][e] = ss[q][e] = 0.f;
+      for (int e = 0; e < 8; ++e) s[q][e] = ss[q][e] = ss2[q][e] = 0.f;
     static_assert(!BNRED || STATS, "the batch-norm backward sums use the statistics epilogue");
+    static_assert(BNRED >= 0 && BNRED <= 2, "no sums, one batch norm's, two batch norms'");
     constexpr int RD = !BNRED ? 1 : (RPF < OP ? RPF : OP);
-    u32x4 ryv[RD];
+    constexpr int RD2 = BNRED == 2 ? RD : 1;
+    u32x4 ryv[RD], ryv2[RD2];
     unsigned rmkv[RD];
-    auto red_fetch = [&](int ps_, u32x4& yv, unsigned& mk) {
+    auto red_fetch = [&](int ps_, u32x4& yv, u32x4& yv2, unsigned& mk) {
       const int row = ps_ * RPO + orow;
       const int m = tile_m * BM + row;
       const u32x4 z4 = {0u, 0u, 0u, 0u};
       yv = z4;
+      if constexpr (BNRED == 2) yv2 = z4;
       mk = 0xffu;
       if (m < p.M && n0 < co8) {
         const size_t ro = row_off(row, m);
         yv = *reinterpret_cast<const u32x4*>(reinterpret_cast<const bf16_t*>(p.red_y) + ro);
+        if constexpr (BNRED == 2) yv2 = *reinterpret_cast<const u32x4*>(reinterpret_cast<const bf16_t*>(p.red_y2) + ro);
         if (p.red_mask) mk = (unsigned)p.red_mask[ro >> 3];
       }
     };
     if constexpr (BNRED) {
 #pragma unroll
-      for (int i = 0; i < RD; ++i) red_fetch(i, ryv[i], rmkv[i]);
+      for (int i = 0; i < RD; ++i) red_fetch(i, ryv[i], ryv2[i % RD2], rmkv[i]);
     }
 #pragma unroll
     for (int ps = 0; ps < OP; ++ps) {
@@ -269,10 +275,10 @@
       }
       const int row = ps * RPO + orow;
       const int m = tile_m * BM + row;
-      u32x4 ry = ryv[ps % RD];
+      u32x4 ry = ryv[ps % RD], ry2 = ryv2[ps % RD2];
       unsigned rmk = rmkv[ps % RD];
       if constexpr (BNRED) {
-        if (ps + RD < OP) red_fetch(ps + RD, ryv[ps % RD], rmkv[ps % RD]);
+        if (ps + RD < OP) red_fetch(ps + RD, ryv[ps % RD], ryv2[ps % RD2], rmkv[ps % RD]);
       }
       u32x4 v = *reinterpret_cast<const u32x4*>(os + row * LDO + oc * 16);
       if (m < p.M && n0 < co8) {
@@ -331,6 +337,12 @@
             s[ps / PPG][e] += dz;
             ss[ps / PPG][e] += dz * fy[e];
           }
+          if constexpr (BNRED == 2) {
+            float fy2[8];
+            unpack8(ry2, fy2);
+#pragma unroll
+            for (int e = 0; e < 8; ++e) ss2[ps / PPG][e] += (((rmk >> e) & 1u) ? f[e] : 0.f) * fy2[e];
+          }
         } else {
 #pragma unroll
           for (int e = 0; e < 8; ++e) {
@@ -342,15 +354,19 @@
     }
     if constexpr (STATS) {
       float* red = reinterpret_cast<float*>(smem);
+      constexpr int NB = BNRED == 2 ? 2 : 1;
+#pragma unroll
+      for (int b = 0; b < NB; ++b)
 #pragma unroll
       for (int q = 0; q < SG; ++q) {
         __syncthreads();
 #pragma unroll
         for (int e = 0; e < 8; ++e) {
           red[(orow * 2 + 0) * BN + oc * 8 + e] = s[q][e];
-          red[(orow * 2 + 1) * BN + oc * 8 + e] = ss[q][e];
+          red[(orow * 2 + 1) * BN + oc * 8 + e] = b ? ss2[q][e] : ss[q][e];
         }
         __syncthreads();
+        float* const out = b ? p.stats2 : p.stats;
         for (int idx = tid; idx < 2 * BN; idx += C::NT) {
           const int which = idx / BN, nl = idx - which * BN;
           float t = 0.f;
@@ -358,7 +374,7 @@
           for (int g = 0; g < RPO; ++g) t += red[(g * 2 + which) * BN + nl];
           const int n = tile_n * BN + nl;
           const int mb = tile_m * SG + q;
-          if (n < p.Co && mb * STATS_BM < p.M) p.stats[((size_t)mb * 2 + which) * p.Co + n] = t;
+          if (n < p.Co && mb * STATS_BM < p.M) out[((size_t)mb * 2 + which) * p.Co + n] = t;
         }
       }
     }
diff --git a/assembled_cnn_amd/lib.py b/assembled_cnn_amd/lib.py
--- a/assembled_cnn_amd/lib.py
+++ b/assembled_cnn_amd/lib.py
@@ -119,7 +119,7 @@
 
 
 ASM_F32, ASM_BF16, ASM_F16 = 0, 1, 2
-ASM_DGRAD_MASKED, ASM_DGRAD_POOLED, ASM_DGRAD_BNRED = 1, 2, 4
+ASM_DGRAD_MASKED, ASM_DGRAD_POOLED, ASM_DGRAD_BNRED, ASM_DGRAD_BNRED2 = 1, 2, 4, 8
 CONV_DGRAD_S2 = 5
 CONV_DENSE = 6
 ASM_AA_SCONV, ASM_AA_PROJ = 1, 2
@@ -153,6 +153,8 @@
     'asm_conv2d_dgrad_pooled': (_I, [_D, _P, _P, _P, _P, _P, _I, _I, _I, _I, _I, _I, _P, _P]),
     'asm_conv2d_dgrad_bnred_blocks': (_I, [_D]),
     'asm_conv2d_dgrad_bnred': (_I, [_D, _P, _P, _P, _P, _P, _P, _P, _P, _P]),
+    'asm_conv2d_dgrad_pooled_bnred_blocks': (_I, [_D, _I]),
+    'asm_conv2d_dgrad_pooled_bnred': (_I, [_D, _P, _P, _P, _P, _P, _I, _I, _I, _I, _I, _I, _P, _P, _P, _P, _P, _P, _P]),
     'asm_conv2d_dgrad_kernel': (_I, [_D, _I]),
     'asm_conv2d_wgrad_workspace_bytes': (_Z, [_D]),
     'asm_conv2d_wgrad': (_I, [_D, _P, _P, _P, _P, _Z, _P]),
diff --git a/assembled_cnn_amd/nn.py b/assembled_cnn_amd/nn.py
--- a/assembled_cnn_amd/nn.py
+++ b/assembled_cnn_amd/nn.py
@@ -281,6 +281,7 @@
 class RedCtx(NamedTuple):
   y: torch.Tensor
   mask: Optional[torch.Tensor]
+  y2: Optional[torch.Tensor] = None
 
 
 class Var(object):
@@ -370,10 +371,15 @@
     pg, self.pool_grad = self.pool_grad, None
     return pg
 
-  def take_red(self, g, relu_mask):
+  def take_red(self, g, relu_mask, dual: bool = False):
     red, self.red = self.red, None
     ok = red is not None and red[1] is g and self.red_ctx is not None and self.red_ctx.mask is relu_mask
-    return red[0] if ok else None
+    if not ok:
+      return None
+    part = red[0]
+    if dual:
+      return part if isinstance(part, tuple) else None
+    return part[0] if isinstance(part, tuple) else part
 
   def park_dy(self, dy):
     self.pre_dy = dy
@@ -567,8 +573,12 @@
     dd = d
     if self.kpad != self.cout:
       dd = ops.make_conv_desc(d.N, d.H, d.W, d.C, self.kpad, d.R, d.S, d.stride, pad=d.pad, Ho=d.Ho, Wo=d.Wo)
-    if red_ctx is not None and pool is None and ops.dgrad_bnred_ok(dd):
-      return ops.conv_dgrad_bnred(dd, dy, a.wt_view(self._wts), addend, addend_mask, red_ctx.y, red_ctx.mask)
+    if red_ctx is not None and pool is None and red_ctx.y2 is None:
+      if ops.dgrad_bnred_ok(dd):
+        return ops.conv_dgrad_bnred(dd, dy, a.wt_view(self._wts), addend, addend_mask, red_ctx.y, red_ctx.mask)
+    elif red_ctx is not None and ops.dgrad_pooled_bnred_ok(dd, pool is not None, red_ctx.y2 is not None):
+      return ops.conv_dgrad_pooled_bnred(dd, dy, a.wt_view(self._wts), addend, addend_mask, pool, red_ctx.y, red_ctx.y2,
+                                         red_ctx.mask)
     return ops.conv_dgrad(dd, dy, a.wt_view(self._wts), addend, addend_mask, pool), None
 
 
@@ -614,7 +624,7 @@
   else:
     apply = 'own'
   offer_red = (taped and ctx.training and apply in ('dual', 'own') and Cn % 8 == 0
-               and not (residual is not None and residual.bn_ctx is not None and dual_bn_on()))
+               and not (residual is not None and residual.bn_ctx is not None and dual_bn_on() and not ops.dgrad_bnred2_on()))
   return ConvBnForm(stats, fold, apply, taped and relu, taped and linear, offer_red)
 
 
@@ -673,7 +683,9 @@
     if form.save_bn:
       out.bn_ctx = saved
   if form.offer_red:
-    out.red_ctx = RedCtx(y, mask_t)
+    sc_bn = residual.bn_ctx if (residual is not None and rm == 1 and relu and dual_bn_on() and lazy_dz_on()) else None
+    dual_red = sc_bn is not None and sc_bn.M == M and sc_bn.C == Cn and residual.needs_grad and ops.dgrad_bnred2_on()
+    out.red_ctx = RedCtx(y, mask_t, sc_bn.y if dual_red else None)
 
   if ctx.tape is not None:
     x_t = x.data
@@ -710,7 +722,8 @@
       elif route == 'dual':
         dy, dy_sc = ops.bn_bwd_dual(dout, y, sc.y, mask_t, M, Cn,
                                     (gamma, mean, invstd, a.g(bn.gamma), a.g(bn.beta)),
-                                    (sc.gamma, sc.mean, sc.invstd, a.g(sc.bn.gamma), a.g(sc.bn.beta)))
+                                    (sc.gamma, sc.mean, sc.invstd, a.g(sc.bn.gamma), a.g(sc.bn.beta)),
+                                    raw_parts=out.take_red(dout, mask_t, dual=True))
         residual.park_dy(dy_sc)
       else:
         dy, dz = ops.bn_bwd(dout, y, bmask, brelu, M, Cn, gamma, mean, invstd, a.g(bn.gamma), a.g(bn.beta),
diff --git a/assembled_cnn_amd/ops.py b/assembled_cnn_amd/ops.py
--- a/assembled_cnn_amd/ops.py
+++ b/assembled_cnn_amd/ops.py
@@ -253,6 +253,44 @@
   if mode == '0' or (mode == '1x1' and d.R != 1):
     return False
   return dgrad_kernel(d, _lib.ASM_DGRAD_BNRED) >= 0
+
+
+_BNRED2_MIN_ROWS = 100000
+
+
+def dgrad_bnred2_on() -> bool:
+  return (knob('ASM_BN_RED', '1') not in ('0', 'nodual')
+          and getattr(L(), 'asm_conv2d_dgrad_pooled_bnred', None) is not None)
+
+
+def dgrad_pooled_bnred_ok(d: ConvDesc, pooled: bool, dual: bool) -> bool:
+  mode = knob('ASM_BN_RED', '1')
+  if mode == '0' or (pooled and mode == 'nopool') or (dual and mode == 'nodual'):
+    return False
+  if getattr(L(), 'asm_conv2d_dgrad_pooled_bnred', None) is None:
+    return False
+  if dual and not pooled and d.N * d.H * d.W < _BNRED2_MIN_ROWS:
+    return False
+  variant = (_lib.ASM_DGRAD_POOLED if pooled else 0) | (_lib.ASM_DGRAD_BNRED2 if dual else _lib.ASM_DGRAD_BNRED)
+  return dgrad_kernel(d, variant) >= 0
+
+
+def conv_dgrad_pooled_bnred(d: ConvDesc, dy: torch.Tensor, wt: torch.Tensor, addend, addend_mask, pool, bn_y: torch.Tensor,
+                            bn_y2, bn_mask):
+  dx = empty((d.N, d.H, d.W, d.C), BF16, dy)
+  variant = (_lib.ASM_DGRAD_POOLED if pool is not None else 0) | (_lib.ASM_DGRAD_BNRED2 if bn_y2 is not None else _lib.ASM_DGRAD_BNRED)
+  blocks = L().asm_conv2d_dgrad_pooled_bnred_blocks(C.byref(d), variant)
+  part = empty((blocks, 2, d.C), F32, dy)
+  part2 = empty((blocks, 2, d.C), F32, dy) if bn_y2 is not None else None
+  pdy, pk, pst, ppad, pcv = pool if pool is not None else (None, 0, 0, 0, 0)
+  pHo, pWo = (pdy.shape[1], pdy.shape[2]) if pdy is not None else (0, 0)
+  ev = _TIMER.start('dgrad', d) if _TIMER is not None else None
+  check(L().asm_conv2d_dgrad_pooled_bnred(C.byref(d), _ptr(dy), _ptr(wt), _ptr(addend), _ptr(addend_mask), _ptr(pdy), pk, pst,
+                                          ppad, pHo, pWo, 1 if pcv else 0, _ptr(bn_y), _ptr(bn_y2), _ptr(bn_mask), _ptr(part),
+                                          _ptr(part2), _ptr(dx), _stream()), 'conv2d_dgrad_pooled_bnred')
+  if ev is not None:
+    ev.record()
+  return dx, (part if part2 is None else (part, part2))
 
 
 def conv_dgrad_bnred(d: ConvDesc, dy: torch.Tensor, wt: torch.Tensor, addend, addend_mask, bn_y: torch.Tensor, bn_mask):
@@ -438,15 +476,18 @@
   return (y, mask) if want_mask else y
 
 
-def bn_bwd_dual(dy, xa, xb, mask, M, Cn, bn_a, bn_b):
-  ev = _bn_ev(M * Cn * (2 * 6.0 + 4.0 + 2 * 0.125))
-  blocks = L().asm_bn_stats_blocks(M, Cn)
-  pa, pb = empty((blocks, 2, Cn), F32, dy), empty((blocks, 2, Cn), F32, dy)
-  check(L().asm_bn_bwd_reduce2(_ptr(dy), _ptr(xa), _ptr(xb), _ptr(mask), M, Cn, _ptr(bn_a[1]), _ptr(bn_a[2]),
-                               _ptr(bn_b[1]), _ptr(bn_b[2]), _ptr(pa), _ptr(pb), _stream()), 'bn_bwd_reduce2')
+def bn_bwd_dual(dy, xa, xb, mask, M, Cn, bn_a, bn_b, raw_parts=None):
+  ev = _bn_ev(M * Cn * ((0.0 if raw_parts is not None else 6.0 + 0.125) + 6.0 + 4.0 + 0.125))
+  if raw_parts is not None:
+    pa, pb = raw_parts
+  else:
+    blocks = L().asm_bn_stats_blocks(M, Cn)
+    pa, pb = empty((blocks, 2, Cn), F32, dy), empty((blocks, 2, Cn), F32, dy)
+    check(L().asm_bn_bwd_reduce2(_ptr(dy), _ptr(xa), _ptr(xb), _ptr(mask), M, Cn, _ptr(bn_a[1]), _ptr(bn_a[2]),
+                                 _ptr(bn_b[1]), _ptr(bn_b[2]), _ptr(pa), _ptr(pb), _stream()), 'bn_bwd_reduce2')
   co = empty((6, Cn), F32, dy)
   for i, (part, (gamma, mean, invstd, dgamma, dbeta)) in enumerate(((pa, bn_a), (pb, bn_b))):
-    _bn_bwd_coeffs(part, M, Cn, gamma, mean, invstd, dgamma, dbeta, co[3 * i:3 * i + 3])
+    _bn_bwd_coeffs(part, M, Cn, gamma, mean, invstd, dgamma, dbeta, co[3 * i:3 * i + 3], raw=raw_parts is not None)
   dxa, dxb = torch.empty_like(xa), torch.empty_like(xb)
   check(L().asm_bn_bwd_apply2(_ptr(dy), _ptr(xa), _ptr(xb), _ptr(mask), M, Cn, _ptr(co), _ptr(dxa), _ptr(dxb), _stream()),
         'bn_bwd_apply2')
diff --git a/include/asm_hip.h b/include/asm_hip.h
--- a/include/asm_hip.h
+++ b/include/asm_hip.h
@@ -82,9 +82,16 @@
                            const uint8_t* addend_mask, const void* bn_y, const uint8_t* bn_relu_mask, float* partial,
                            void* dx, void* stream);
 
+int asm_conv2d_dgrad_pooled_bnred_blocks(const asm_conv_desc* d, int variant);
+int asm_conv2d_dgrad_pooled_bnred(const asm_conv_desc* d, const void* dy, const void* wt, const void* addend,
+                                  const uint8_t* addend_mask, const void* pool_dy, int pool_k, int pool_stride, int pool_pad,
+                                  int pool_Ho, int pool_Wo, int count_valid, const void* bn_y, const void* bn_y2,
+                                  const uint8_t* bn_relu_mask, float* partial, float* partial2, void* dx, void* stream);
+
 #define ASM_DGRAD_MASKED 1
 #define ASM_DGRAD_POOLED 2
 #define ASM_DGRAD_BNRED 4
+#define ASM_DGRAD_BNRED2 8
 int asm_conv2d_dgrad_kernel(const asm_conv_desc* d, int variant);
 
 size_t asm_conv2d_wgrad_workspace_bytes(const asm_conv_desc* d);
```

Result: no change. 10910 images/sec, median of 6 (+0.7%).
